# lenskit/lkpy

Hardware: AMD Instinct MI355X
Metric: ALS-implicit epochs/sec (ML-25M-shaped, k=64) (higher is better)
Workload: dtype f32; 1 GPU; MovieLens-25M-shaped, als-implicit k=64, 829 timed epochs, 1 x MI355X; solver=cholesky, n_items=62423, nnz=25000095, parallelism=single GPU

## Files before the change

### lkpy_amd/csrc/als_cg.hip

```cpp
#include "als_plan.h"
#include "common.h"

namespace lk {

template <int FPL>
struct Vec {
    float v[FPL];
};

template <int FPL>
__device__ __forceinline__ Vec<FPL> vload(const float *p)
{
    Vec<FPL> r;
    if constexpr (FPL == 1) {
        r.v[0] = p[0];
    } else if constexpr (FPL == 2) {
        f32x2 t = *reinterpret_cast<const f32x2 *>(p);
        r.v[0] = t.x;
        r.v[1] = t.y;
    } else {
        f32x4 t = *reinterpret_cast<const f32x4 *>(p);
        r.v[0] = t.x;
        r.v[1] = t.y;
        r.v[2] = t.z;
        r.v[3] = t.w;
    }
    return r;
}

template <int CTRL>
__device__ __forceinline__ float cg_dpp(float x)
{
    return __builtin_bit_cast(
        float, __builtin_amdgcn_update_dpp(0, __builtin_bit_cast(int, x), CTRL, 0xf, 0xf, false));
}
__device__ __forceinline__ float cg_wave_sum(float x)
{
    x += cg_dpp<0xB1>(x);
    x += cg_dpp<0x4E>(x);
    x += cg_dpp<0x141>(x);
    x += cg_dpp<0x140>(x);
    return (bcast(x, 0) + bcast(x, 16)) + (bcast(x, 32) + bcast(x, 48));
}
template <int FPL>
__device__ __forceinline__ float vdot(const Vec<FPL> &a, const Vec<FPL> &b)
{
    float s = 0.f;
#pragma unroll
    for (int c = 0; c < FPL; ++c) s = fmaf(a.v[c], b.v[c], s);
    return cg_wave_sum(s);
}

__device__ __forceinline__ int64_t cg_uniform64(int64_t v)
{
    const unsigned lo = __builtin_amdgcn_readfirstlane((unsigned)v);
    const unsigned hi = __builtin_amdgcn_readfirstlane((unsigned)((unsigned long long)v >> 32));
    return (int64_t)(((unsigned long long)hi << 32) | lo);
}

__device__ __forceinline__ float cg_reduce8(const float (&a)[8], int lane)
{
    const bool b0 = lane & 1, b1 = lane & 2, b2 = lane & 4;
    float b[4], c[2];
#pragma unroll
    for (int m = 0; m < 4; ++m) {
        const float keep = b0 ? a[m + 4] : a[m], send = b0 ? a[m] : a[m + 4];
        b[m] = keep + cg_dpp<0xB1>(send);
    }
#pragma unroll
    for (int m = 0; m < 2; ++m) {
        const float keep = b1 ? b[m + 2] : b[m], send = b1 ? b[m] : b[m + 2];
        c[m] = keep + cg_dpp<0x4E>(send);
    }
    const float keep = b2 ? c[1] : c[0], send = b2 ? c[0] : c[1];
    float d = keep + __shfl_xor(send, 4, 64);
    d += cg_dpp<0x128>(d);
    d += __shfl_xor(d, 16, 64);
    d += __shfl_xor(d, 32, 64);
    return d;
}
#define CG_REV3(j) ((((j) & 1) << 2) | ((j) & 2) | (((j) & 4) >> 2))

template <int KP, bool IS64, int NW>
__global__ __launch_bounds__(256, (NW == 1 && KP <= 128) ? 3 : 2) void als_cg_kernel(
    const typename IndPtr<IS64>::type *__restrict__ indptr, const int32_t *__restrict__ indices,
    const float *__restrict__ values, const int32_t *__restrict__ order, int64_t n_rows,
    const float *__restrict__ other, float *__restrict__ this_, const float *__restrict__ otor,
    int ld_otor, int k, float tol, int max_iter, float *__restrict__ row_delta,
    int *__restrict__ status, TaskCtlDev ctl, int64_t t_begin, int64_t t_end)
{
    static_assert(NW == 4 || NW == 1, "NW");
    constexpr int FPL = KP / 64;
    constexpr bool OTOR_LDS = KP <= 128;
    constexpr int GB = 8;
    constexpr int RI = 64 / FPL;
    constexpr int NG = RI / GB;
    constexpr int TB = FPL <= 2 ? 16 : 8;
    __shared__ float part[4][KP];
    extern __shared__ __attribute__((aligned(16))) float otor_s[];
    const int wave_in_wg = __builtin_amdgcn_readfirstlane(threadIdx.x >> 6);
    const int wave = NW == 4 ? wave_in_wg : 0;
    const bool lead = NW == 1 || wave_in_wg == 0;
    const int lane = lane_id();
    const int f0 = lane * FPL;
    auto team_sync = [&]() {
        if constexpr (NW == 4) __syncthreads();
    };
    const int myj = CG_REV3(lane & 7);
    if (OTOR_LDS) {
        for (int e = threadIdx.x; e < KP * KP; e += 256) {
            const int g = e / KP, f = e % KP;
            otor_s[e] = (g < k && f < k) ? otor[(int64_t)g * ld_otor + f] : 0.f;
        }
        __syncthreads();
    }

    __shared__ int s_cancel;
    (void)n_rows;
    for (int64_t t = t_begin + (NW == 4 ? (int64_t)blockIdx.x : (int64_t)blockIdx.x * 4 + wave_in_wg);
         t < t_end; t += (NW == 4 ? (int64_t)gridDim.x : (int64_t)gridDim.x * 4)) {
        if (NW == 4 && ctl.d_cancel) {
            if (threadIdx.x == 0) s_cancel = ctl_cancelled(ctl, (blockIdx.x & 31) == 0) ? 1 : 0;
            __syncthreads();
            const int c = s_cancel;
            __syncthreads();
            if (c) return;
        }
        const int row = __builtin_amdgcn_readfirstlane(order[t]);
        const int64_t beg = cg_uniform64(indptr[row]), end = cg_uniform64(indptr[row + 1]);
        float *xrow = this_ + (int64_t)row * KP;
        if (end == beg) {
            if (lead)
#pragma unroll
                for (int c = 0; c < FPL; ++c) xrow[f0 + c] = 0.f;
            if (lead && lane == 0) row_delta[row] = 0.f;
            if (ctl.d_done && lead && lane == 0) ctl_advance(ctl, 1);
            continue;
        }
        const int64_t n = end - beg;
        const int share = n >= NW * RI ? RI : (int)((n + NW * GB - 1) / (NW * GB)) * GB;
        const int64_t rbeg = beg + (int64_t)wave * share;
        int nres = (int)(end - rbeg < share ? end - rbeg : share);
        nres = __builtin_amdgcn_readfirstlane(nres < 0 ? 0 : nres);
        const int64_t sbeg = beg + NW * (int64_t)share;
        Vec<FPL> qres[RI];
        float vg[NG];
        const int myitem = indices[lane < nres ? rbeg + lane : beg];
#pragma unroll
        for (int g = 0; g < NG; ++g) {
            vg[g] = 0.f;
            if (g * GB < nres) {
                vg[g] = (g * GB + myj < nres) ? values[rbeg + g * GB + myj] : 0.f;
#pragma unroll
                for (int j = 0; j < GB; ++j) {
                    const int i = g * GB + j;
                    const int64_t it = __builtin_amdgcn_readlane(myitem, i);
                    qres[i] = vload<FPL>(other + it * KP + f0);
                    if (i >= nres)
#pragma unroll
                        for (int c = 0; c < FPL; ++c) qres[i].v[c] = 0.f;
                }
            } else {
#pragma unroll
                for (int j = 0; j < GB; ++j)
#pragma unroll
                    for (int c = 0; c < FPL; ++c) qres[g * GB + j].v[c] = 0.f;
            }
        }
        auto apply = [&](const Vec<FPL> &p, Vec<FPL> &out) {
            Vec<FPL> u;
#pragma unroll
            for (int c = 0; c < FPL; ++c) u.v[c] = 0.f;
#pragma unroll
            for (int g2 = 0; g2 < NG; g2 += 2) {
                if (g2 * GB < nres) {
                    float a[2][GB];
#pragma unroll
                    for (int h = 0; h < 2; ++h)
#pragma unroll
                        for (int j = 0; j < GB; ++j) {
                            float sacc = 0.f;
#pragma unroll
                            for (int c = 0; c < FPL; ++c)
                                sacc = fmaf(qres[(g2 + h) * GB + j].v[c], p.v[c], sacc);
                            a[h][j] = sacc;
                        }
                    float coefv[2];
#pragma unroll
                    for (int h = 0; h < 2; ++h) coefv[h] = vg[g2 + h] * cg_reduce8(a[h], lane);
#pragma unroll
                    for (int h = 0; h < 2; ++h)
#pragma unroll
                        for (int j = 0; j < GB; ++j) {
                            const float coef = bcast(coefv[h], CG_REV3(j));
#pragma unroll
                            for (int c = 0; c < FPL; ++c)
                                u.v[c] = fmaf(coef, qres[(g2 + h) * GB + j].v[c], u.v[c]);
                        }
                }
            }
            for (int64_t e0 = sbeg + (int64_t)wave * TB; e0 < end; e0 += NW * TB) {
                Vec<FPL> q[TB];
                const int tailitem = indices[(lane < TB && e0 + lane < end) ? e0 + lane : beg];
                float vmine[TB / GB];
#pragma unroll
                for (int h = 0; h < TB / GB; ++h)
                    vmine[h] = (e0 + h * GB + myj < end) ? values[e0 + h * GB + myj] : 0.f;
#pragma unroll
                for (int j = 0; j < TB; ++j) {
                    const int64_t it = __builtin_amdgcn_readlane(tailitem, j);
                    q[j] = vload<FPL>(other + it * KP + f0);
                }
#pragma unroll
                for (int h = 0; h < TB / GB; ++h) {
                    float a[GB];
#pragma unroll
                    for (int j = 0; j < GB; ++j) {
                        float sacc = 0.f;
#pragma unroll
                        for (int c = 0; c < FPL; ++c) sacc = fmaf(q[h * GB + j].v[c], p.v[c], sacc);
                        a[j] = sacc;
                    }
                    const float coefv = vmine[h] * cg_reduce8(a, lane);
#pragma unroll
                    for (int j = 0; j < GB; ++j) {
                        const float coef = bcast(coefv, CG_REV3(j));
#pragma unroll
                        for (int c = 0; c < FPL; ++c)
                            u.v[c] = fmaf(coef, q[h * GB + j].v[c], u.v[c]);
                    }
                }
            }
#pragma unroll 8
            for (int gi = 0; gi < KP / NW; ++gi) {
                const int g = wave * (KP / NW) + gi;
                if (!OTOR_LDS && g >= k) continue;
                float pg = 0.f;
#pragma unroll
                for (int c = 0; c < FPL; ++c)
                    if ((g % FPL) == c) pg = bcast(p.v[c], g / FPL);
                if (OTOR_LDS) {
                    const Vec<FPL> o = vload<FPL>(&otor_s[g * KP + f0]);
#pragma unroll
                    for (int c = 0; c < FPL; ++c) u.v[c] = fmaf(pg, o.v[c], u.v[c]);
                } else {
#pragma unroll
                    for (int c = 0; c < FPL; ++c) {
                        const int f = f0 + c;
                        const float o = (f < k) ? otor[(int64_t)g * ld_otor + f] : 0.f;
                        u.v[c] = fmaf(pg, o, u.v[c]);
                    }
                }
            }
            if constexpr (NW == 1) {
                out = u;
            } else {
                __syncthreads();
#pragma unroll
                for (int c = 0; c < FPL; ++c) part[wave][f0 + c] = u.v[c];
                __syncthreads();
#pragma unroll
                for (int c = 0; c < FPL; ++c)
                    out.v[c] = ((part[0][f0 + c] + part[1][f0 + c]) + part[2][f0 + c]) +
                               part[3][f0 + c];
            }
        };

        Vec<FPL> y, d;
        {
            Vec<FPL> yw, dw;
#pragma unroll
            for (int c = 0; c < FPL; ++c) yw.v[c] = dw.v[c] = 0.f;
#pragma unroll
            for (int g = 0; g < NG; ++g) {
                if (g * GB < nres) {
#pragma unroll
                    for (int j = 0; j < GB; ++j) {
                        const float val = bcast(vg[g], CG_REV3(j));
#pragma unroll
                        for (int c = 0; c < FPL; ++c) {
                            const float qc = qres[g * GB + j].v[c];
                            yw.v[c] = fmaf(val + 1.0f, qc, yw.v[c]);
                            dw.v[c] = fmaf(val * qc, qc, dw.v[c]);
                        }
                    }
                }
            }
            for (int64_t e0 = sbeg + (int64_t)wave * GB; e0 < end; e0 += NW * GB) {
                Vec<FPL> q[GB];
                float val[GB];
                const bool mine = lane < GB && e0 + lane < end;
                const int tailitem = indices[mine ? e0 + lane : beg];
                const float tailval = mine ? values[e0 + lane] : -1.0f;
#pragma unroll
                for (int j = 0; j < GB; ++j) {
                    const bool in = e0 + j < end;
                    const int64_t it = __builtin_amdgcn_readlane(tailitem, j);
                    val[j] = bcast(tailval, j);
                    q[j] = vload<FPL>(other + it * KP + f0);
                    if (!in)
#pragma unroll
                        for (int c = 0; c < FPL; ++c) q[j].v[c] = 0.f;
                }
#pragma unroll
                for (int j = 0; j < GB; ++j)
#pragma unroll
                    for (int c = 0; c < FPL; ++c) {
                        yw.v[c] = fmaf(val[j] + 1.0f, q[j].v[c], yw.v[c]);
                        dw.v[c] = fmaf(val[j] * q[j].v[c], q[j].v[c], dw.v[c]);
                    }
            }
            if constexpr (NW == 1) {
#pragma unroll
                for (int c = 0; c < FPL; ++c) {
                    const int f = f0 + c;
                    const float od = (f < k) ? otor[(int64_t)f * ld_otor + f] : 1.0f;
                    y.v[c] = yw.v[c];
                    d.v[c] = od + dw.v[c];
                }
            } else {
                __syncthreads();
#pragma unroll
                for (int c = 0; c < FPL; ++c) part[wave][f0 + c] = yw.v[c];
                __syncthreads();
#pragma unroll
                for (int c = 0; c < FPL; ++c)
                    y.v[c] = ((part[0][f0 + c] + part[1][f0 + c]) + part[2][f0 + c]) +
                             part[3][f0 + c];
                __syncthreads();
#pragma unroll
                for (int c = 0; c < FPL; ++c) part[wave][f0 + c] = dw.v[c];
                __syncthreads();
#pragma unroll
                for (int c = 0; c < FPL; ++c) {
                    const int f = f0 + c;
                    const float od = (f < k) ? otor[(int64_t)f * ld_otor + f] : 1.0f;
                    d.v[c] = od + (((part[0][f] + part[1][f]) + part[2][f]) + part[3][f]);
                }
            }
        }
        Vec<FPL> dinv;
#pragma unroll
        for (int c = 0; c < FPL; ++c) dinv.v[c] = 1.0f / d.v[c];
        Vec<FPL> x, xold, r, z, p, ap;
#pragma unroll
        for (int c = 0; c < FPL; ++c) xold.v[c] = x.v[c] = xrow[f0 + c];
        apply(x, ap);
        const float ynorm2 = vdot<FPL>(y, y);
#pragma unroll
        for (int c = 0; c < FPL; ++c) {
            r.v[c] = y.v[c] - ap.v[c];
            z.v[c] = r.v[c] * dinv.v[c];
            p.v[c] = z.v[c];
        }
        float rz = vdot<FPL>(r, z);
        float rr = vdot<FPL>(r, r);
        const float stop = tol * tol * ynorm2;
        int it = 0;
        bool bad = !(ynorm2 == ynorm2);
        while (it < max_iter && rr > stop && !bad) {
            apply(p, ap);
            const float pap = vdot<FPL>(p, ap);
            if (!(pap > 0.f)) {
                bad = true;
                break;
            }
            const float alpha = rz / pap;
#pragma unroll
            for (int c = 0; c < FPL; ++c) {
                x.v[c] = fmaf(alpha, p.v[c], x.v[c]);
                r.v[c] = fmaf(-alpha, ap.v[c], r.v[c]);
                z.v[c] = r.v[c] * dinv.v[c];
            }
            const float rz_new = vdot<FPL>(r, z);
            rr = vdot<FPL>(r, r);
            const float beta = rz_new / rz;
            rz = rz_new;
#pragma unroll
            for (int c = 0; c < FPL; ++c) p.v[c] = fmaf(beta, p.v[c], z.v[c]);
            ++it;
        }
        float dd = 0.f;
#pragma unroll
        for (int c = 0; c < FPL; ++c) {
            const float df = (f0 + c < k) ? x.v[c] - xold.v[c] : 0.f;
            dd = fmaf(df, df, dd);
            bad = bad || !(fabsf(x.v[c]) <= 3.0e38f);
        }
        dd = cg_wave_sum(dd);
        if (lead) {
#pragma unroll
            for (int c = 0; c < FPL; ++c) xrow[f0 + c] = (f0 + c < k) ? x.v[c] : 0.f;
            if (lane == 0) row_delta[row] = dd;
        }
        if (__any(bad) && lead && lane == 0) atomicCAS(status, 0, row + 1);
        if (lead && lane == 0) {
            atomicAdd(&status[2], it);
            atomicAdd(&status[3], 1);
        }
        if (ctl.d_done && lead && lane == 0) ctl_advance(ctl, 1);
        team_sync();
    }
}

template <int KP, bool IS64>
static int launch_cg(const lk_als_plan *p, const void *indptr, const int32_t *indices,
                     const float *values, int64_t n_rows, int k, float *this_,
                     const float *other, const float *otor, int ld_otor, char *ws,
                     float *out_frob, hipStream_t st, int64_t t_begin)
{
    using IT = typename IndPtr<IS64>::type;
    int *status = reinterpret_cast<int *>(ws + p->off_status);
    float *row_delta = reinterpret_cast<float *>(ws + p->off_delta);
    float *partial = reinterpret_cast<float *>(ws + p->off_partial);
    if (t_begin == 0) LK_HIP_CHECK(hipMemsetAsync(status, 0, 64, st));
    if (p->ctl) {
        LK_HIP_CHECK(hipMemsetAsync(row_delta, 0, (size_t)n_rows * sizeof(float), st));
        int rc = ctl_begin(p->ctl, n_rows, n_rows, st);
        if (rc != LK_OK) return rc;
    }
    const int max_iter = p->cg_max_iter > 0 ? p->cg_max_iter : k;
    int64_t t_w1 = p->ctl ? n_rows : p->t_cg1;
    if (t_w1 < t_begin) t_w1 = t_begin;
    const size_t lds = KP <= 128 ? (size_t)KP * KP * sizeof(float) : 0;
    auto k4 = als_cg_kernel<KP, IS64, 4>;
    auto k1 = als_cg_kernel<KP, IS64, 1>;
    if (lds > 0) {
        LK_HIP_CHECK(hipFuncSetAttribute(reinterpret_cast<const void *>(k4),
                                         hipFuncAttributeMaxDynamicSharedMemorySize, (int)lds));
        LK_HIP_CHECK(hipFuncSetAttribute(reinterpret_cast<const void *>(k1),
                                         hipFuncAttributeMaxDynamicSharedMemorySize, (int)lds));
    }
    if (t_w1 > t_begin) {
        const int64_t n4 = t_w1 - t_begin;
        const int64_t blocks = n4 < 256 * 8 ? n4 : 256 * 8;
        hipLaunchKernelGGL(k4, dim3((unsigned)blocks), dim3(256), lds, st,
                           static_cast<const IT *>(indptr), indices, values, p->d_order, n_rows,
                           other, this_, otor, ld_otor, k, p->cg_tol, max_iter, row_delta,
                           status, p->ctl ? p->ctl->dev() : TaskCtlDev{}, t_begin, t_w1);
    }
    if (n_rows > t_w1) {
        const int64_t n1 = (n_rows - t_w1 + 3) / 4;
        const int64_t blocks = n1 < 256 * 8 ? n1 : 256 * 8;
        hipLaunchKernelGGL(k1, dim3((unsigned)blocks), dim3(256), lds, st,
                           static_cast<const IT *>(indptr), indices, values, p->d_order, n_rows,
                           other, this_, otor, ld_otor, k, p->cg_tol, max_iter, row_delta,
                           status, TaskCtlDev{}, t_w1, n_rows);
    }
    return launch_delta_reduce(row_delta, n_rows, partial, out_frob, st);
}

int als_cg_half_epoch(const lk_als_plan *p, const void *indptr, int is64, const int32_t *indices,
                      const float *values, int64_t n_rows, int k, float *this_, int ld_this,
                      const float *other, int ld_other, const float *otor, int ld_otor, char *ws,
                      float *out_frob, hipStream_t st)
{
    int64_t t_begin = 0;
    const int64_t t_exact = p->ctl ? 0 : p->cg_exact;
    if (t_exact > 0) {
        p->dense_limit = t_exact;
        const int rc =
            p->KP > 64 ? als_blk_half_epoch(p, indptr, is64, indices, values, n_rows, 0, k, this_,
                                            other, otor, ld_otor, ws, out_frob, st, false, 0.f)
                       : als_chol_half_epoch(p, indptr, is64, indices, values, n_rows, k, this_,
                                             ld_this, other, ld_other, otor, ld_otor, ws, out_frob,
                                             st, false, 0.f);
        p->dense_limit = -1;
        if (rc != LK_OK) return rc;
        t_begin = t_exact;
    }
#define LK_CG_CASE(KPV)                                                                     \
    return is64 ? launch_cg<KPV, true>(p, indptr, indices, values, n_rows, k, this_, other, \
                                       otor, ld_otor, ws, out_frob, st, t_begin)            \
                : launch_cg<KPV, false>(p, indptr, indices, values, n_rows, k, this_, other, \
                                        otor, ld_otor, ws, out_frob, st, t_begin)
    switch (p->KP) {
        case 64: LK_CG_CASE(64);
        case 128: LK_CG_CASE(128);
        case 256: LK_CG_CASE(256);
    }
#undef LK_CG_CASE
    set_error("CG solver: unsupported padded embedding size %d (needs k > 32)", p->KP);
    return LK_E_INVALID;
}

}

extern "C" int lk_als_plan_cg_stats(const lk_als_plan *plan, void *d_ws, void *stream,
                                    int64_t *out_iterations, int64_t *out_rows)
{
    LK_REQUIRE(plan && d_ws, "lk_als_plan_cg_stats: null pointer");
    int st[4] = {0, 0, 0, 0};
    LK_HIP_CHECK(hipMemcpyAsync(st, static_cast<char *>(d_ws) + plan->off_status, sizeof(st),
                                hipMemcpyDeviceToHost, lk::as_stream(stream)));
    LK_HIP_CHECK(hipStreamSynchronize(lk::as_stream(stream)));
    if (out_iterations) *out_iterations = st[2];
    if (out_rows) *out_rows = st[3];
    return LK_OK;
}
```

### lkpy_amd/csrc/als_chol.hip

```cpp
#include <algorithm>
#include <utility>

#include "als_plan.h"
#include "common.h"
#include "delta_reduce.h"

#ifndef LK_ALS_RING
#define LK_ALS_RING 4
#endif

namespace lk {

#ifdef LK_ALS_PHASES
__device__ unsigned *lk_als_phase_buf;
#define LK_PHASE_T(var) const unsigned long long var = __builtin_amdgcn_s_memtime()
#define LK_PHASE_ADD(i, a, b) \
    if (lane_id() == 0 && lk_als_phase_buf) lk_als_phase_buf[t * 8 + (i)] = (unsigned)((b) - (a))
#else
#define LK_PHASE_T(var)
#define LK_PHASE_ADD(i, a, b)
#endif

__host__ __device__ constexpr int als_tiles(int NT) { return NT * (NT + 1) / 2; }
__host__ __device__ constexpr int tidx(int ti, int tj) { return tj * (tj + 1) / 2 + ti; }

template <int NT>
struct Gram {
    f32x4 t[als_tiles(NT)];
    float y[NT];
    float yc = 0.f;
};

__device__ __forceinline__ void swap32(float &a, float &b)
{
    asm volatile("s_nop 1\n\tv_permlane32_swap_b32 %0, %1" : "+v"(a), "+v"(b));
}
__device__ __forceinline__ void swap16(float &a, float &b)
{
    asm volatile("s_nop 1\n\tv_permlane16_swap_b32 %0, %1" : "+v"(a), "+v"(b));
}

template <int NT>
__device__ __forceinline__ void y_chain_step(float &yc, const float (&q)[NT], const float v1)
{
    float p[4];
#pragma unroll
    for (int t = 0; t < 4; ++t) p[t] = t < NT ? __fmul_rn(q[t < NT ? t : 0], v1) : 0.f;
    swap32(p[0], p[2]);
    swap32(p[1], p[3]);
    swap16(p[0], p[1]);
    swap16(p[2], p[3]);
    yc = __fadd_rn(yc, p[0]);
    yc = __fadd_rn(yc, p[1]);
    yc = __fadd_rn(yc, p[2]);
    yc = __fadd_rn(yc, p[3]);
}

template <int NT>
__device__ __forceinline__ void load_q(const float *p, float (&q)[NT])
{
    if constexpr (NT == 1) {
        q[0] = *p;
    } else if constexpr (NT == 2) {
        f32x2 t = *reinterpret_cast<const f32x2 *>(p);
        q[0] = t.x;
        q[1] = t.y;
    } else {
        static_assert(NT == 4, "Cholesky path supports NT in {1,2,4}");
        f32x4 t = *reinterpret_cast<const f32x4 *>(p);
        q[0] = t.x;
        q[1] = t.y;
        q[2] = t.z;
        q[3] = t.w;
    }
}

template <int NT>
struct GatherRing {
    static constexpr int RING = LK_ALS_RING;
    float q[RING][NT];
    float v[RING];
};

template <int NT>
__device__ __forceinline__ void ring_issue(GatherRing<NT> &R, const int slot_idx, const int g,
                                           const float *stage_slot,
                                           const float *__restrict__ other)
{
    constexpr int KP = NT * 16;
    const int lane = lane_id();
    const int col = __builtin_bit_cast(int, stage_slot[g * 4]);
    R.v[slot_idx] = stage_slot[64 + g * 4];
    load_q<NT>(other + (int64_t)col * KP + (lane & 15) * NT, R.q[slot_idx]);
}

template <int NT, bool MASKED, bool SEQY = false, bool WITH_Y = true>
__device__ __forceinline__ void ring_consume(Gram<NT> &G, const GatherRing<NT> &R,
                                             const int slot_idx, const int g, const int nb,
                                             const bool expl)
{
    const int lane = lane_id();
    const bool live = !MASKED || (g * 4 + (lane >> 4)) < nb;
    const float v = R.v[slot_idx];
    const float va = expl ? 1.0f : v;
    float q[NT], a[NT];
#pragma unroll
    for (int t = 0; t < NT; ++t) {
        q[t] = live ? R.q[slot_idx][t] : 0.f;
        a[t] = q[t] * va;
    }
#pragma unroll
    for (int tj = 0; tj < NT; ++tj)
#pragma unroll
        for (int ti = 0; ti <= tj; ++ti)
            G.t[tidx(ti, tj)] = __builtin_amdgcn_mfma_f32_16x16x4f32(a[ti], q[tj],
                                                                     G.t[tidx(ti, tj)], 0, 0, 0);
    if constexpr (WITH_Y) {
        const float v1 = expl ? v : v + 1.0f;
        if constexpr (SEQY) {
            y_chain_step<NT>(G.yc, q, v1);
        } else {
#pragma unroll
            for (int t = 0; t < NT; ++t) G.y[t] = fmaf(q[t], v1, G.y[t]);
        }
    }
}

constexpr int GRAM_STAGE_WORDS = 256;

template <int NT, bool SEQY = false, bool WITH_Y = true>
__device__ __forceinline__ void gram_accumulate(Gram<NT> &G, const int32_t *__restrict__ cols,
                                                const float *__restrict__ vals, int64_t beg,
                                                int64_t end, const float *__restrict__ other,
                                                int , const bool expl,
                                                float *stage )
{
    const int lane = lane_id();
    constexpr int RING = GatherRing<NT>::RING;
    static_assert(RING >= 1 && RING <= 8 && 16 % RING == 0, "gather ring: 1, 2, 4 or 8 slots");
    GatherRing<NT> R;
    const int64_t last = end - 1;

    float *wr_cur = stage + lane, *wr_nxt = stage + 128 + lane;
    const float *rd_cur = stage + (lane >> 4), *rd_nxt = stage + 128 + (lane >> 4);
    int nxt_col;
    float nxt_val;
    {
        const int64_t e = (beg + lane < end) ? beg + lane : last;
        wr_cur[0] = __builtin_bit_cast(float, cols[e]);
        wr_cur[64] = vals[e];
    }
#pragma unroll
    for (int g = 0; g < RING; ++g) ring_issue<NT>(R, g, g, rd_cur, other);

    int64_t base = beg;
    for (; base + 64 <= end; base += 64) {
        {
            const int64_t e = (base + 64 + lane < end) ? base + 64 + lane : last;
            nxt_col = cols[e];
            nxt_val = vals[e];
        }
#pragma unroll
        for (int g = 0; g < 16; ++g) {
            ring_consume<NT, false, SEQY, WITH_Y>(G, R, g % RING, g, 64, expl);
            if (g == 16 - RING - 2) {
                wr_nxt[0] = __builtin_bit_cast(float, nxt_col);
                wr_nxt[64] = nxt_val;
            }
            if (g < 16 - RING)
                ring_issue<NT>(R, g % RING, g + RING, rd_cur, other);
            else
                ring_issue<NT>(R, g % RING, g + RING - 16, rd_nxt, other);
            __builtin_amdgcn_sched_barrier(0);
        }
        float *tw = wr_cur;
        wr_cur = wr_nxt;
        wr_nxt = tw;
        const float *tr = rd_cur;
        rd_cur = rd_nxt;
        rd_nxt = tr;
    }
    if (base < end) {
        const int nb = (int)(end - base);
        const int ngroups = (nb + 3) >> 2;
#pragma unroll
        for (int g = 0; g < 16; ++g) {
            if (g < ngroups) ring_consume<NT, true, SEQY, WITH_Y>(G, R, g % RING, g, nb, expl);
            if (g < 16 - RING) ring_issue<NT>(R, g % RING, g + RING, rd_cur, other);
        }
    }
}

#ifndef LK_ALS_DMA_RING
#define LK_ALS_DMA_RING 8
#endif
constexpr int DMA_RING = LK_ALS_DMA_RING;

template <int N>
__device__ __forceinline__ void wait_vm()
{
    asm volatile("s_waitcnt vmcnt(%0)" ::"n"(N) : "memory");
}
__device__ __forceinline__ void wait_vm_upto(const int n)
{
    if (n >= 7) wait_vm<7>();
    else if (n == 6) wait_vm<6>();
    else if (n == 5) wait_vm<5>();
    else if (n == 4) wait_vm<4>();
    else if (n == 3) wait_vm<3>();
    else if (n == 2) wait_vm<2>();
    else if (n == 1) wait_vm<1>();
    else wait_vm<0>();
}

__device__ __forceinline__ void dma_issue(const unsigned ring_lds, const int slot_idx, const int g,
                                          const float *stage_slot,
                                          const float *__restrict__ other)
{
    const int lane = lane_id();
    const unsigned col = __builtin_bit_cast(unsigned, stage_slot[g * 4]);
    const uint64_t lane_base = (uint64_t)(uintptr_t)(other + (lane & 15) * 4);
    const float *src = reinterpret_cast<const float *>(lane_base + (uint64_t)col * 256ull);
    const unsigned dst = ring_lds + slot_idx * 1024;
    unsigned keep;
    asm volatile(
        "s_mov_b32 %0, m0\n\ts_mov_b32 m0, %2\n\ts_nop 0\n\t"
        "global_load_lds_dwordx4 %1, off\n\ts_mov_b32 m0, %0"
        : "=&s"(keep)
        : "v"(src), "s"(dst)
        : "memory");
}

struct DmaOperand {
    f32x4 q;
    float v;
};
__device__ __forceinline__ DmaOperand dma_fetch(const float *ring, const int slot_idx, const int g,
                                                const float *stage_slot)
{
    DmaOperand o;
    o.q = *reinterpret_cast<const f32x4 *>(ring + slot_idx * 256 + lane_id() * 4);
    o.v = stage_slot[64 + g * 4];
    return o;
}

template <bool MASKED, bool SEQY = false, bool WITH_Y = true>
__device__ __forceinline__ void dma_apply(Gram<4> &G, const DmaOperand &o, const int g,
                                          const int nb, const bool expl)
{
    const int lane = lane_id();
    const bool live = !MASKED || (g * 4 + (lane >> 4)) < nb;
    const float v = o.v;
    const float va = expl ? 1.0f : v;
    float q[4] = {o.q.x, o.q.y, o.q.z, o.q.w}, a[4];
#pragma unroll
    for (int t = 0; t < 4; ++t) {
        q[t] = live ? q[t] : 0.f;
        a[t] = q[t] * va;
    }
#pragma unroll
    for (int tj = 0; tj < 4; ++tj)
#pragma unroll
        for (int ti = 0; ti <= tj; ++ti)
            G.t[tidx(ti, tj)] = __builtin_amdgcn_mfma_f32_16x16x4f32(a[ti], q[tj],
                                                                     G.t[tidx(ti, tj)], 0, 0, 0);
    if constexpr (WITH_Y) {
        const float v1 = expl ? v : v + 1.0f;
        if constexpr (SEQY) {
            y_chain_step<4>(G.yc, q, v1);
        } else {
#pragma unroll
            for (int t = 0; t < 4; ++t) G.y[t] = fmaf(q[t], v1, G.y[t]);
        }
    }
}

template <bool MASKED, bool SEQY = false, bool WITH_Y = true>
__device__ __forceinline__ void dma_consume(Gram<4> &G, const float *ring, const int slot_idx,
                                            const int g, const int nb, const float *stage_slot,
                                            const bool expl)
{
    dma_apply<MASKED, SEQY, WITH_Y>(G, dma_fetch(ring, slot_idx, g, stage_slot), g, nb, expl);
}

template <int NT>
__host__ __device__ constexpr int slab_floats();
template <int NT, bool WITH_Y = true>
__device__ __forceinline__ void slab_store(const Gram<NT> &G, float *__restrict__ slab);
template <int NT, bool WITH_Y = true>
__device__ __forceinline__ void gram_zero(Gram<NT> &G);

template <bool SEQY = false, bool WITH_Y = true, int RING = DMA_RING>
__device__ __forceinline__ void gram_accumulate_dma(Gram<4> &G, const int32_t *__restrict__ cols,
                                                    const float *__restrict__ vals, int64_t beg,
                                                    int64_t end, const float *__restrict__ other,
                                                    const bool expl, float *ring, float *stage,
                                                    float *__restrict__ slab = nullptr)
{
    static_assert(RING == 8 || RING == 4, "DMA ring: 4 or 8 groups");
    const int lane = lane_id();
    const int64_t last = end - 1;
    const unsigned ring_lds =
        __builtin_amdgcn_readfirstlane((unsigned)(uintptr_t) reinterpret_cast<void *>(ring));

    float *wr_cur = stage + lane, *wr_nxt = stage + 128 + lane;
    const float *rd_cur = stage + (lane >> 4), *rd_nxt = stage + 128 + (lane >> 4);
    {
        const int64_t e = (beg + lane < end) ? beg + lane : last;
        wr_cur[0] = __builtin_bit_cast(float, cols[e]);
        wr_cur[64] = vals[e];
    }
    const int total = (int)((end - beg + 3) >> 2);
#pragma unroll
    for (int g = 0; g < RING; ++g)
        if (g < total) dma_issue(ring_lds, g, g, rd_cur, other);

    int64_t base = beg;
    int g0 = 0;
    for (; g0 + 16 + RING <= total; base += 64, g0 += 16) {
        int nxt_col;
        float nxt_val;
        {
            const int64_t e = (base + 64 + lane < end) ? base + 64 + lane : last;
            nxt_col = cols[e];
            nxt_val = vals[e];
        }
        wait_vm<RING - 1>();
        DmaOperand cur = dma_fetch(ring, 0, 0, rd_cur);
#pragma unroll
        for (int g = 0; g < 16; ++g) {
            DmaOperand nxt = cur;
            if (g + 1 < 16) {
                wait_vm<RING - 2>();
                nxt = dma_fetch(ring, (g + 1) % RING, g + 1, rd_cur);
            }
            dma_apply<false, SEQY, WITH_Y>(G, cur, g, 64, expl);
            if (g == 16 - RING - 2) {
                wr_nxt[0] = __builtin_bit_cast(float, nxt_col);
                wr_nxt[64] = nxt_val;
            }
            if (g < 16 - RING)
                dma_issue(ring_lds, g % RING, g + RING, rd_cur, other);
            else
                dma_issue(ring_lds, g % RING, g + RING - 16, rd_nxt, other);
            cur = nxt;
            __builtin_amdgcn_sched_barrier(0);
        }
        if (slab && ((g0 + 16) & 63) == 0) {
            slab_store<4, WITH_Y>(G, slab);
            slab += slab_floats<4>();
            gram_zero<4, WITH_Y>(G);
        }
        float *tw = wr_cur;
        wr_cur = wr_nxt;
        wr_nxt = tw;
        const float *tr = rd_cur;
        rd_cur = rd_nxt;
        rd_nxt = tr;
    }
    for (; g0 < total; base += 64, g0 += 16) {
        const int nb = (int)((end - base < 64) ? end - base : 64);
        const bool more = g0 + 16 < total;
        int nxt_col = 0;
        float nxt_val = 0.f;
        if (more) {
            const int64_t e = (base + 64 + lane < end) ? base + 64 + lane : last;
            nxt_col = cols[e];
            nxt_val = vals[e];
        }
#pragma unroll
        for (int g = 0; g < 16; ++g) {
            const int gg = g0 + g;
            if (gg < total) {
                const int later = total - 1 - gg;
                wait_vm_upto(later < RING - 1 ? later : RING - 1);
                dma_consume<true, SEQY, WITH_Y>(G, ring, g % RING, g, nb, rd_cur, expl);
            }
            if (g == 16 - RING - 2 && more) {
                wr_nxt[0] = __builtin_bit_cast(float, nxt_col);
                wr_nxt[64] = nxt_val;
            }
            if (gg + RING < total) {
                if (g < 16 - RING)
                    dma_issue(ring_lds, g % RING, g + RING, rd_cur, other);
                else
                    dma_issue(ring_lds, g % RING, g + RING - 16, rd_nxt, other);
            }
        }
        if (slab && ((g0 + 16) & 63) == 0 && g0 + 16 < total) {
            slab_store<4, WITH_Y>(G, slab);
            slab += slab_floats<4>();
            gram_zero<4, WITH_Y>(G);
        }
        float *tw = wr_cur;
        wr_cur = wr_nxt;
        wr_nxt = tw;
        const float *tr = rd_cur;
        rd_cur = rd_nxt;
        rd_nxt = tr;
    }
}

template <bool WITH_Y = true, int RING = DMA_RING>
__device__ __forceinline__ void gram_accumulate_dma_256(Gram<4> &G, const int32_t *__restrict__ cols,
                                                        const float *__restrict__ vals, int64_t beg,
                                                        const float *__restrict__ other,
                                                        const bool expl, float *ring, float *stage)
{
    constexpr int TOTAL = 64;
    const int lane = lane_id();
    const unsigned ring_lds =
        __builtin_amdgcn_readfirstlane((unsigned)(uintptr_t) reinterpret_cast<void *>(ring));
    float *const wr0 = stage + lane, *const wr1 = stage + 128 + lane;
    const float *const rd0 = stage + (lane >> 4), *const rd1 = stage + 128 + (lane >> 4);
    wr0[0] = __builtin_bit_cast(float, cols[beg + lane]);
    wr0[64] = vals[beg + lane];
#pragma unroll
    for (int g = 0; g < RING; ++g) dma_issue(ring_lds, g, g, rd0, other);
#pragma unroll
    for (int b = 0; b < 4; ++b) {
        float *const wr_nxt = (b & 1) ? wr0 : wr1;
        const float *const rd_cur = (b & 1) ? rd1 : rd0, *const rd_nxt = (b & 1) ? rd0 : rd1;
        int nxt_col = 0;
        float nxt_val = 0.f;
        if (b < 3) {
            nxt_col = cols[beg + 64 * (b + 1) + lane];
            nxt_val = vals[beg + 64 * (b + 1) + lane];
        }
        {
            const int later = TOTAL - 1 - 16 * b;
            wait_vm_upto(later < RING - 1 ? later : RING - 1);
        }
        DmaOperand cur = dma_fetch(ring, 0, 0, rd_cur);
#pragma unroll
        for (int g = 0; g < 16; ++g) {
            const int gg = 16 * b + g;
            DmaOperand nxt = cur;
            if (g + 1 < 16) {
                const int later = TOTAL - 1 - (gg + 1);
                const int issued_after = (gg + RING < TOTAL ? gg + RING - 1 : TOTAL - 1) - (gg + 1);
                wait_vm_upto(issued_after < later ? issued_after : later);
                nxt = dma_fetch(ring, (g + 1) % RING, g + 1, rd_cur);
            }
            dma_apply<false, false, WITH_Y>(G, cur, g, 64, expl);
            if (g == 16 - RING - 2 && b < 3) {
                wr_nxt[0] = __builtin_bit_cast(float, nxt_col);
                wr_nxt[64] = nxt_val;
            }
            if (gg + RING < TOTAL) {
                if (g < 16 - RING)
                    dma_issue(ring_lds, g % RING, g + RING, rd_cur, other);
                else
                    dma_issue(ring_lds, g % RING, g + RING - 16, rd_nxt, other);
            }
            cur = nxt;
            __builtin_amdgcn_sched_barrier(0);
        }
    }
}

template <int NT>
__host__ __device__ constexpr int slab_floats()
{
    return (als_tiles(NT) * 4 + NT) * 64;
}

template <int NT, bool WITH_Y>
__device__ __forceinline__ void slab_store(const Gram<NT> &G, float *__restrict__ slab)
{
    const int lane = lane_id();
#pragma unroll
    for (int e = 0; e < als_tiles(NT); ++e)
        __builtin_nontemporal_store(G.t[e], reinterpret_cast<f32x4 *>(slab + (e * 64 + lane) * 4));
    if constexpr (WITH_Y) {
#pragma unroll
        for (int t = 0; t < NT; ++t) slab[als_tiles(NT) * 256 + lane * NT + t] = G.y[t];
    }
}

template <int NT, bool WITH_Y = true>
__device__ __forceinline__ void slab_add(Gram<NT> &G, const float *__restrict__ slab)
{
    const int lane = lane_id();
#pragma unroll
    for (int e = 0; e < als_tiles(NT); ++e)
        G.t[e] += *reinterpret_cast<const f32x4 *>(slab + (e * 64 + lane) * 4);
    if constexpr (WITH_Y) {
#pragma unroll
        for (int t = 0; t < NT; ++t) G.y[t] += slab[als_tiles(NT) * 256 + lane * NT + t];
    }
}

template <int NT, bool WITH_Y>
__device__ __forceinline__ void gram_zero(Gram<NT> &G)
{
#pragma unroll
    for (int e = 0; e < als_tiles(NT); ++e) G.t[e] = f32x4{0.f, 0.f, 0.f, 0.f};
    if constexpr (WITH_Y) {
#pragma unroll
        for (int t = 0; t < NT; ++t) G.y[t] = 0.f;
    }
}

__global__ __launch_bounds__(256) void slab_group_reduce_kernel(float *__restrict__ slabs,
                                                                int64_t slab_floats,
                                                                int64_t sum_floats,
                                                                const int32_t *__restrict__ grp_head,
                                                                const int32_t *__restrict__ grp_cnt,
                                                                int parts)
{
    const int g = blockIdx.x / parts;
    const int64_t e = ((int64_t)(blockIdx.x - g * parts) * 256 + threadIdx.x) * 4;
    if (e >= sum_floats) return;
    float *head = slabs + (size_t)grp_head[g] * slab_floats + e;
    const int cnt = grp_cnt[g];
    f32x4 acc = *reinterpret_cast<const f32x4 *>(head);
    int c = 1;
    for (; c + 8 <= cnt; c += 8) {
        f32x4 v[8];
#pragma unroll
        for (int u = 0; u < 8; ++u)
            v[u] = __builtin_nontemporal_load(
                reinterpret_cast<const f32x4 *>(head + (size_t)(c + u) * slab_floats));
#pragma unroll
        for (int u = 0; u < 8; ++u) acc += v[u];
    }
    for (; c < cnt; ++c)
        acc += *reinterpret_cast<const f32x4 *>(head + (size_t)c * slab_floats);
    *reinterpret_cast<f32x4 *>(head) = acc;
}

int launch_slab_group_reduce(const lk_als_plan *p, float *slabs, size_t slab_floats, hipStream_t st,
                             size_t sum_floats)
{
    if (p->n_groups <= 0) return LK_OK;
    if (sum_floats == 0) sum_floats = slab_floats;
    const int parts = (int)((sum_floats / 4 + 255) / 256);
    hipLaunchKernelGGL(slab_group_reduce_kernel, dim3((unsigned)(p->n_groups * parts)), dim3(256),
                       0, st, slabs, (int64_t)slab_floats, (int64_t)sum_floats, p->d_grp_head,
                       p->d_grp_cnt, parts);
    LK_HIP_CHECK(hipGetLastError());
    return LK_OK;
}

#ifndef LK_ALS_CHUNK_RING
#define LK_ALS_CHUNK_RING 8
#endif
constexpr int CHUNK_RING = LK_ALS_CHUNK_RING;

template <int NT>
__host__ __device__ constexpr int chunk_lds_floats()
{
    return GRAM_STAGE_WORDS + (NT == 4 ? CHUNK_RING * 256 : 0);
}

int als_chol_chunk_wgs_per_cu()
{
    const int by_lds = (int)(160 * 1024 / (4 * chunk_lds_floats<4>() * sizeof(float)));
    return by_lds < 5 ? by_lds : 5;
}

template <int NT, bool EXPL, bool WITH_Y>
__device__ __forceinline__ void als_chunk_body(
    const int32_t *__restrict__ indices, const float *__restrict__ values,
    const int64_t *__restrict__ chunk_beg, const int32_t *__restrict__ chunk_len,
    int64_t n_chunks, const float *__restrict__ other, int ld, float *__restrict__ slabs,
    const int64_t blk, float *__restrict__ lds_flat,
    const int32_t *__restrict__ chunk_slab = nullptr, const int block_len = 0)
{
    constexpr bool DMA = NT == 4;
    float(*stage_all)[chunk_lds_floats<NT>()] =
        reinterpret_cast<float(*)[chunk_lds_floats<NT>()]>(lds_flat);
    const int wave = __builtin_amdgcn_readfirstlane(threadIdx.x >> 6);
    const int64_t c = blk * 4 + wave;
    if (c >= n_chunks) return;
    Gram<NT> G;
    gram_zero<NT, WITH_Y>(G);
    const int64_t beg = chunk_beg[c];
    float *slab = slabs + (size_t)(chunk_slab ? chunk_slab[c] : c) * slab_floats<NT>();
    if constexpr (DMA) {
        const int len = chunk_len[c];
        if (block_len == 256 && len > 256) {
            gram_accumulate_dma<false, WITH_Y, CHUNK_RING>(
                G, indices, values, beg, beg + len, other, EXPL,
                stage_all[wave] + GRAM_STAGE_WORDS, stage_all[wave], slab);
            slab += (size_t)((len - 1) >> 8) * slab_floats<NT>();
        } else if (len == 256)
            gram_accumulate_dma_256<WITH_Y, CHUNK_RING>(
                G, indices, values, beg, other, EXPL, stage_all[wave] + GRAM_STAGE_WORDS,
                stage_all[wave]);
        else
            gram_accumulate_dma<false, WITH_Y, CHUNK_RING>(
                G, indices, values, beg, beg + len, other, EXPL,
                stage_all[wave] + GRAM_STAGE_WORDS, stage_all[wave]);
    } else
        gram_accumulate<NT, false, WITH_Y>(G, indices, values, beg, beg + chunk_len[c], other, ld,
                                           EXPL, stage_all[wave]);
    slab_store<NT, WITH_Y>(G, slab);
}

template <int NT, bool EXPL, bool WITH_Y>
__global__ __launch_bounds__(256) void als_chunk_kernel(
    const int32_t *__restrict__ indices, const float *__restrict__ values,
    const int64_t *__restrict__ chunk_beg, const int32_t *__restrict__ chunk_len,
    int64_t n_chunks, const float *__restrict__ other, int ld, float *__restrict__ slabs,
    const int32_t *__restrict__ chunk_slab, int block_len)
{
    __shared__ __attribute__((aligned(16))) float lds_flat[4 * chunk_lds_floats<NT>()];
    als_chunk_body<NT, EXPL, WITH_Y>(indices, values, chunk_beg, chunk_len, n_chunks, other, ld,
                                     slabs, (int64_t)blockIdx.x, lds_flat, chunk_slab, block_len);
}

template <int KP>
struct LPack {
    __host__ __device__ static constexpr int c0(int j) { return (j + 1) & ~3; }
    __host__ __device__ static constexpr int off(int j)
    {
        const int m = j >> 2, r = j & 3;
        return 4 * KP * m - 8 * m * m + 4 * m + r * (KP - 4 * m);
    }
    static constexpr int SIZE = KP * KP / 2 + KP;
};

template <int NT>
__host__ __device__ constexpr int hybrid_lds_floats()
{
    return LPack<NT * 16>::SIZE + NT * 16 + 256;
}

template <int NT, int M>
__device__ __forceinline__ void hybrid_step(Gram<NT> &G, float &b, float &minpiv,
                                            float *__restrict__ lds, const int lane)
{
    constexpr int KP = NT * 16, J = 4 * M, TJ = M >> 2, MG = M & 3;
    using P = LPack<KP>;
    const int slot = lane >> 4;
    float *rinvarr = lds + P::SIZE;
    float *scr = rinvarr + KP;

#pragma unroll
    for (int t = TJ; t < NT; ++t)
        if (slot == MG)
            *reinterpret_cast<f32x4 *>(&scr[(t * 16 + (lane & 15)) * 4]) = G.t[tidx(TJ, t)];
    f32x4 pv = f32x4{0.f, 0.f, 0.f, 0.f};
    if (slot >= TJ && lane < KP) pv = *reinterpret_cast<const f32x4 *>(&scr[lane * 4]);
    float pr[4] = {pv.x, pv.y, pv.z, pv.w};

    float lp[4];
#pragma unroll
    for (int s0 = 0; s0 < 4; ++s0) {
        const int j = J + s0;
        const float piv = bcast(pr[s0], j);
        minpiv = fminf(minpiv, piv);
        const float rinv = __builtin_amdgcn_rsqf(piv);
        rinvarr[j] = rinv;
        const float lj = (lane > j) ? pr[s0] * rinv : 0.f;
        if (j + 1 < KP) {
            const bool in = lane >= P::c0(j) && lane < KP;
            float *dst = in ? &lds[P::off(j) + lane - P::c0(j)] : &scr[lane];
            *dst = lj;
        }
        const float zj = bcast(b, j) * rinv;
        b = fmaf(-lj, zj, b);
#pragma unroll
        for (int s = s0 + 1; s < 4; ++s) pr[s] = fmaf(-lj, bcast(lj, J + s), pr[s]);
        lp[s0] = lj;
    }
    if constexpr (J + 4 < KP) {
        swap32(lp[0], lp[2]);
        swap32(lp[1], lp[3]);
        swap16(lp[0], lp[1]);
        swap16(lp[2], lp[3]);
        float nq[NT];
#pragma unroll
        for (int t = TJ; t < NT; ++t) nq[t] = -lp[t];
#pragma unroll
        for (int ti = TJ; ti < NT; ++ti)
#pragma unroll
            for (int t2 = ti; t2 < NT; ++t2)
                G.t[tidx(ti, t2)] = __builtin_amdgcn_mfma_f32_16x16x4f32(
                    nq[ti], lp[t2], G.t[tidx(ti, t2)], 0, 0, 0);
    }
}

template <int NT, int... Ms>
__device__ __forceinline__ void hybrid_steps(Gram<NT> &G, float &b, float &minpiv,
                                             float *__restrict__ lds, const int lane,
                                             std::integer_sequence<int, Ms...>)
{
    (hybrid_step<NT, Ms>(G, b, minpiv, lds, lane), ...);
}

template <int NT>
__device__ __forceinline__ float hybrid_solve(Gram<NT> &G, float &b, float *__restrict__ lds
#ifdef LK_ALS_PHASES
                                              ,
                                              unsigned long long *tmid
#endif
)
{
    constexpr int KP = NT * 16;
    using P = LPack<KP>;
    int lane = lane_id();
    asm volatile("" : "+v"(lane));
    b = 0.f;
#pragma unroll
    for (int tt = 0; tt < NT; ++tt) b = ((lane >> 4) == tt) ? G.y[tt] : b;
    float minpiv = 3.0e38f;
    hybrid_steps<NT>(G, b, minpiv, lds, lane, std::make_integer_sequence<int, KP / 4>{});
#ifdef LK_ALS_PHASES
    asm volatile("" : "+v"(b));
    *tmid = __builtin_amdgcn_s_memtime();
#endif
    const float dinv = (lane < KP) ? lds[P::SIZE + lane] : 0.f;
    b *= dinv;
    const int my_c0 = (lane + 1) & ~3;
    const float *mycol = lds + P::off(lane) - my_c0;
#pragma unroll
    for (int j4 = KP / 4 - 1; j4 >= 0; --j4) {
        f32x4 l4 = f32x4{0.f, 0.f, 0.f, 0.f};
        if (lane < KP - 1 && 4 * j4 >= my_c0) l4 = *reinterpret_cast<const f32x4 *>(mycol + 4 * j4);
#pragma unroll
        for (int u = 3; u >= 0; --u) {
            const int j = 4 * j4 + u;
            if (j >= 1) {
                const float xj = bcast(b * dinv, j);
                b = fmaf(-l4[u], xj, b);
            }
        }
    }
    b *= dinv;
    return minpiv;
}

template <int NT, bool IS64, bool EXPL, bool CTL, bool YREF = false, bool SEQY = false>
__device__ __forceinline__ void als_solve_body(
    const typename IndPtr<IS64>::type *__restrict__ indptr, const int32_t *__restrict__ indices,
    const float *__restrict__ values, const int32_t *__restrict__ order, int64_t n_rows,
    const int32_t *__restrict__ row_slab, const float *__restrict__ other, int ld_other,
    float *__restrict__ this_, int ld_this, const float *__restrict__ otor_p,
    const float *__restrict__ slabs, float *__restrict__ row_delta, int *__restrict__ status,
    int k, float reg, TaskCtlDev ctl, const float *__restrict__ y_ref, int chunk_rt,
    const int64_t blk, float *__restrict__ lds_flat)
{
    constexpr int KP = NT * 16;
    float(*lds_all)[hybrid_lds_floats<NT>()] =
        reinterpret_cast<float(*)[hybrid_lds_floats<NT>()]>(lds_flat);

    const int wave = __builtin_amdgcn_readfirstlane(threadIdx.x >> 6);
    const int lane = lane_id();
    const int sub = lane & 15, slot = lane >> 4;
    const int64_t t = blk * 4 + wave;
    if (t >= n_rows) return;
    LK_PHASE_T(ph0);
    if constexpr (CTL) {
        int c = 0;
        if (lane == 0) c = ctl_cancelled(ctl, (blk & 63) == 0 && wave == 0) ? 1 : 0;
        if (__builtin_amdgcn_readfirstlane(c)) return;
    }
    const int row = order[t];
    const int64_t beg = indptr[row], end = indptr[row + 1];
    float *lds = lds_all[wave];

    const int my_f = (lane & 15) * NT + (lane >> 4);
    const bool my_valid = (lane < KP) && (my_f < k);
    float *xrow = this_ + (int64_t)row * ld_this;

    if (end == beg) {
        if (lane < KP) xrow[lane] = 0.f;
        if (lane == 0) row_delta[row] = 0.f;
        if constexpr (CTL)
            if (lane == 0) ctl_advance(ctl, 1);
        return;
    }

    LK_PHASE_T(ph1);
    Gram<NT> G;
#pragma unroll
    for (int tj = 0; tj < NT; ++tj)
#pragma unroll
        for (int ti = 0; ti <= tj; ++ti)
#pragma unroll
            for (int r = 0; r < 4; ++r)
                G.t[tidx(ti, tj)][r] = otor_p[(ti * 16 + slot * 4 + r) * KP + tj * 16 + sub];
#pragma unroll
    for (int tt = 0; tt < NT; ++tt) G.y[tt] = 0.f;

    const int first_slab = row_slab[row];
    if (first_slab >= 0) {
        const int64_t n = end - beg;
        const bool refo = YREF && chunk_rt > 0;
        const int ch = refo ? chunk_rt : LK_ALS_CHUNK;
        const int ns = (int)((n + ch - 1) / ch);
        const int step = refo ? ns : (ns > LK_ALS_SLAB_GROUP ? LK_ALS_SLAB_GROUP : 1);
        for (int s = 0; s < ns; s += step)
            slab_add<NT, !YREF>(G, slabs + (size_t)(first_slab + s) * slab_floats<NT>());
    } else {
        if constexpr (NT == 4)
            gram_accumulate_dma<SEQY && !YREF>(G, indices, values, beg, end, other, EXPL, lds,
                                               lds + LPack<KP>::SIZE + KP);
        else
            gram_accumulate<NT, SEQY && !YREF>(G, indices, values, beg, end, other, ld_other,
                                               EXPL, lds);
    }
    if (EXPL) {
        const float dg = reg * (float)(end - beg);
#pragma unroll
        for (int ti = 0; ti < NT; ++ti)
#pragma unroll
            for (int r = 0; r < 4; ++r)
                if (slot * 4 + r == sub && (slot * 4 + r) * NT + ti < k) G.t[tidx(ti, ti)][r] += dg;
    }

#ifdef LK_ALS_PHASES
    asm volatile("" : "+v"(G.t[0]), "+v"(G.t[als_tiles(NT) - 1]));
#endif
    LK_PHASE_T(ph2);
    if (SEQY && !YREF && first_slab < 0) {
#pragma unroll
        for (int tt = 0; tt < NT; ++tt) G.y[tt] = __shfl(G.yc, sub + 16 * tt, 64);
    } else {
#pragma unroll
        for (int tt = 0; tt < NT; ++tt) {
            G.y[tt] += __shfl_xor(G.y[tt], 16, 64);
            G.y[tt] += __shfl_xor(G.y[tt], 32, 64);
        }
    }
    if constexpr (YREF) {
#pragma unroll
        for (int tt = 0; tt < NT; ++tt) G.y[tt] = y_ref[(int64_t)t * KP + sub * NT + tt];
    }
    const float old = my_valid ? xrow[my_f] : 0.f;
    float b;
#ifdef LK_ALS_PHASES
    LK_PHASE_T(ph3);
    unsigned long long ph4 = 0;
    const float minpiv = hybrid_solve<NT>(G, b, lds, &ph4);
    asm volatile("" : "+v"(b));
    LK_PHASE_T(ph5);
#else
    const float minpiv = hybrid_solve<NT>(G, b, lds);
#endif
    const bool bad = !(minpiv > 0.f) || (my_valid && !(fabsf(b) <= 3.0e38f));
    if (__any(bad) && lane == 0) atomicCAS(status, 0, row + 1);

    float d = 0.f;
    if (my_valid) {
        xrow[my_f] = b;
        d = b - old;
    }
    const float d2 = wave_sum(d * d);
    if (lane == 0) row_delta[row] = d2;
    if constexpr (CTL)
        if (lane == 0) ctl_advance(ctl, 1);
#ifdef LK_ALS_PHASES
    LK_PHASE_T(ph6);
    LK_PHASE_ADD(0, ph0, ph1);
    LK_PHASE_ADD(1, ph1, ph2);
    LK_PHASE_ADD(2, ph2, ph3);
    LK_PHASE_ADD(3, ph3, ph4);
    LK_PHASE_ADD(4, ph4, ph5);
    LK_PHASE_ADD(5, ph5, ph6);
    LK_PHASE_ADD(6, (unsigned long long)beg, (unsigned long long)end);
    LK_PHASE_ADD(7, ph0, ph6);
#endif
}

template <int NT, bool IS64, bool EXPL, bool CTL, bool YREF = false, bool SEQY = false>
__global__ __launch_bounds__(256) __attribute__((amdgpu_waves_per_eu(4))) void als_solve_kernel(
    const typename IndPtr<IS64>::type *__restrict__ indptr, const int32_t *__restrict__ indices,
    const float *__restrict__ values, const int32_t *__restrict__ order, int64_t n_rows,
    const int32_t *__restrict__ row_slab, const float *__restrict__ other, int ld_other,
    float *__restrict__ this_, int ld_this, const float *__restrict__ otor_p,
    const float *__restrict__ slabs, float *__restrict__ row_delta, int *__restrict__ status,
    int k, float reg, TaskCtlDev ctl, const float *__restrict__ y_ref = nullptr,
    int chunk_rt = 0)
{
    __shared__ __attribute__((aligned(16))) float lds_flat[4 * hybrid_lds_floats<NT>()];
    als_solve_body<NT, IS64, EXPL, CTL, YREF, SEQY>(indptr, indices, values, order, n_rows,
                                                    row_slab, other, ld_other, this_, ld_this,
                                                    otor_p, slabs, row_delta, status, k, reg, ctl,
                                                    y_ref, chunk_rt, (int64_t)blockIdx.x, lds_flat);
}

template <int CTRL>
__device__ __forceinline__ float wb_dpp_add(float x)
{
    const int y = __builtin_amdgcn_update_dpp(0, __builtin_bit_cast(int, x), CTRL, 0xf, 0xf, false);
    return x + __builtin_bit_cast(float, y);
}
__device__ __forceinline__ float wb_row16_sum(float x)
{
    x = wb_dpp_add<0xB1>(x);
    x = wb_dpp_add<0x4E>(x);
    x = wb_dpp_add<0x141>(x);
    x = wb_dpp_add<0x140>(x);
    return x;
}

template <int KP, bool IS64>
__global__ __launch_bounds__(256) void als_wb64_kernel(
    const typename IndPtr<IS64>::type *__restrict__ indptr, const int32_t *__restrict__ indices,
    const float *__restrict__ values, const int32_t *__restrict__ order, int64_t n_tasks,
    const float *__restrict__ other, const float *__restrict__ z, float *__restrict__ this_,
    float *__restrict__ row_delta, int *__restrict__ status)
{
    constexpr int QF = KP / 4;
    constexpr int NQ = QF / 4;
    __shared__ __attribute__((aligned(16))) float lds_all[4][hybrid_lds_floats<4>()];
    const int wave = __builtin_amdgcn_readfirstlane(threadIdx.x >> 6);
    const int lane = lane_id();
    const int s = lane >> 4, c = lane & 15;
    const int64_t task = (int64_t)blockIdx.x * 4 + wave;
    if (task >= n_tasks) return;
    if (status[1] != 0) return;
    const int row = order[task];
    const int64_t beg = indptr[row], end = indptr[row + 1];
    const int n = (int)(end - beg);
    float *xrow = this_ + (int64_t)row * KP;
    float *lds = lds_all[wave];
    const int nte = __builtin_amdgcn_readfirstlane((n + 15) >> 4);

    const float *mrow[4], *zrow[4];
    float w[4], sv[4];
#pragma unroll
    for (int t = 0; t < 4; ++t) {
        const int el = 16 * t + c;
        const int64_t e = beg + (el < n ? el : n - 1);
        const int col = indices[e];
        const float v = el < n ? values[e] : 0.f;
        w[t] = el < n ? v + 1.0f : 0.f;
        sv[t] = __builtin_sqrtf(v);
        mrow[t] = other + (int64_t)col * KP + 4 * s;
        zrow[t] = z + (int64_t)col * KP + 4 * s;
    }
    f32x4 acc[4][4];
#pragma unroll
    for (int ti = 0; ti < 4; ++ti)
#pragma unroll
        for (int tj = 0; tj < 4; ++tj) acc[ti][tj] = f32x4{0.f, 0.f, 0.f, 0.f};
    for (int q = 0; q < NQ; ++q) {
        f32x4 mq[4], zq[4];
#pragma unroll
        for (int t = 0; t < 4; ++t) {
            mq[t] = f32x4{0.f, 0.f, 0.f, 0.f};
            zq[t] = f32x4{0.f, 0.f, 0.f, 0.f};
            if (t < nte) {
                mq[t] = *reinterpret_cast<const f32x4 *>(mrow[t] + 16 * q);
                zq[t] = *reinterpret_cast<const f32x4 *>(zrow[t] + 16 * q);
            }
        }
#pragma unroll
        for (int ti = 0; ti < 4; ++ti)
#pragma unroll
            for (int tj = 0; tj < 4; ++tj)
                if (ti < nte && tj < nte) {
#pragma unroll
                    for (int el = 0; el < 4; ++el)
                        acc[ti][tj] = __builtin_amdgcn_mfma_f32_16x16x4f32(
                            mq[ti][el], zq[tj][el], acc[ti][tj], 0, 0, 0);
                }
    }
    float b;
    float minpiv;
    auto build = [&](auto &G, auto ntc) {
        constexpr int NTS = decltype(ntc)::value;
#pragma unroll
        for (int ti = 0; ti < NTS; ++ti) {
            float svr[4], rhs[4];
#pragma unroll
            for (int r = 0; r < 4; ++r) {
                svr[r] = __shfl(sv[ti], 4 * s + r, 64);
                float r0 = 0.f;
#pragma unroll
                for (int tj = 0; tj < NTS; ++tj) r0 += wb_row16_sum(acc[ti][tj][r] * w[tj]);
                rhs[r] = svr[r] * r0;
            }
#pragma unroll
            for (int tj = ti; tj < NTS; ++tj)
#pragma unroll
                for (int r = 0; r < 4; ++r)
                    G.t[tidx(ti, tj)][r] = svr[r] * sv[tj] * acc[ti][tj][r] +
                                           ((ti == tj && (4 * s + r) == c) ? 1.0f : 0.f);
            float sel = rhs[0];
            sel = (c & 3) == 1 ? rhs[1] : sel;
            sel = (c & 3) == 2 ? rhs[2] : sel;
            sel = (c & 3) == 3 ? rhs[3] : sel;
            G.y[ti] = __shfl(sel, (c >> 2) * 16 + c, 64);
        }
    };
#ifdef LK_ALS_PHASES
    unsigned long long tmid_unused = 0;
#endif
    if (nte <= 2) {
        Gram<2> G;
        build(G, std::integral_constant<int, 2>{});
#ifdef LK_ALS_PHASES
        minpiv = hybrid_solve<2>(G, b, lds, &tmid_unused);
#else
        minpiv = hybrid_solve<2>(G, b, lds);
#endif
    } else {
        Gram<4> G;
        build(G, std::integral_constant<int, 4>{});
#ifdef LK_ALS_PHASES
        minpiv = hybrid_solve<4>(G, b, lds, &tmid_unused);
#else
        minpiv = hybrid_solve<4>(G, b, lds);
#endif
    }
    float g[4];
    bool bad = !(minpiv > 0.f);
#pragma unroll
    for (int t = 0; t < 4; ++t) {
        g[t] = t < nte ? w[t] - sv[t] * __shfl(b, 16 * t + c, 64) : 0.f;
        bad = bad || !(fabsf(g[t]) <= 3.0e38f);
    }
    if (__any(bad) && lane == 0) atomicCAS(status, 0, row + 1);
    float d2 = 0.f;
    for (int q = 0; q < NQ; ++q) {
        f32x4 a4 = f32x4{0.f, 0.f, 0.f, 0.f};
#pragma unroll
        for (int t = 0; t < 4; ++t)
            if (t < nte) {
                const f32x4 zq = *reinterpret_cast<const f32x4 *>(zrow[t] + 16 * q);
                a4.x = fmaf(g[t], zq.x, a4.x);
                a4.y = fmaf(g[t], zq.y, a4.y);
                a4.z = fmaf(g[t], zq.z, a4.z);
                a4.w = fmaf(g[t], zq.w, a4.w);
            }
        f32x4 xs;
        xs.x = wb_row16_sum(a4.x);
        xs.y = wb_row16_sum(a4.y);
        xs.z = wb_row16_sum(a4.z);
        xs.w = wb_row16_sum(a4.w);
        if (c == 0) {
            f32x4 *dst = reinterpret_cast<f32x4 *>(xrow + 4 * s + 16 * q);
            const f32x4 old = *dst;
            *dst = xs;
            const f32x4 d = xs - old;
            d2 += d.x * d.x + d.y * d.y + d.z * d.z + d.w * d.w;
        }
    }
    d2 = wave_sum(d2);
    if (lane == 0) row_delta[row] = d2;
}

int als_wb64_launch(const lk_als_plan *p, const void *indptr, int is64, const int32_t *indices,
                    const float *values, int64_t t0, int64_t t1, float *this_,
                    const float *other, const float *z, float *row_delta, int *status,
                    hipStream_t st)
{
    const int64_t n = t1 - t0;
    if (n <= 0) return LK_OK;
    const dim3 grid((unsigned)((n + 3) / 4)), block(256);
#define LK_WB64(KPV, IS)                                                                        \
    hipLaunchKernelGGL((als_wb64_kernel<KPV, IS>), grid, block, 0, st,                          \
                       static_cast<const typename IndPtr<IS>::type *>(indptr), indices, values, \
                       p->d_order + t0, n, other, z, this_, row_delta, status)
    if (p->KP == 256) {
        if (is64)
            LK_WB64(256, true);
        else
            LK_WB64(256, false);
    } else if (p->KP == 128) {
        if (is64)
            LK_WB64(128, true);
        else
            LK_WB64(128, false);
    } else {
        set_error("Woodbury row solve: unsupported padded embedding size %d", p->KP);
        return LK_E_INVALID;
    }
#undef LK_WB64
    LK_HIP_CHECK(hipGetLastError());
    return LK_OK;
}

template <int NT>
__global__ void als_prep_otor_kernel(const float *__restrict__ otor, int ld_otor, int k,
                                     float *__restrict__ otor_p)
{
    constexpr int KP = NT * 16;
    int idx = blockIdx.x * blockDim.x + threadIdx.x;
    if (idx >= KP * KP) return;
    int pr = idx / KP, pc = idx % KP;
    int fr = (pr & 15) * NT + (pr >> 4), fc = (pc & 15) * NT + (pc >> 4);
    float v;
    if (fr < k && fc < k)
        v = otor ? otor[fr * ld_otor + fc] : 0.f;
    else
        v = (pr == pc) ? 1.0f : 0.0f;
    otor_p[idx] = v;
}

__global__ void delta_partial_kernel(const float *__restrict__ row_delta, int64_t n,
                                     float *__restrict__ partial)
{
    __shared__ float sm[256];
    delta_partial_body(row_delta, n, (int)gridDim.x, (int)blockIdx.x, sm, partial);
}

__global__ void delta_final_kernel(const float *__restrict__ partial, int n,
                                   float *__restrict__ out)
{
    __shared__ float sm[256];
    delta_final_body(partial, n, sm, out);
}

constexpr int DELTA_BLOCKS = LK_DELTA_BLOCKS;

int launch_delta_reduce(const float *row_delta, int64_t n_rows, float *partial, float *out_frob,
                        hipStream_t st)
{
    hipLaunchKernelGGL(delta_partial_kernel, dim3(DELTA_BLOCKS), dim3(256), 0, st, row_delta,
                       n_rows, partial);
    hipLaunchKernelGGL(delta_final_kernel, dim3(1), dim3(256), 0, st, partial, DELTA_BLOCKS,
                       out_frob);
    LK_HIP_CHECK(hipGetLastError());
    return LK_OK;
}

template <int NT, bool IS64, bool EXPL>
struct CholKind {};

struct CholHalf {
    const lk_als_plan *p;
    const void *indptr;
    bool is64;
    const int32_t *indices;
    const float *values;
    int64_t n_rows;
    int k;
    float *this_;
    int ld_this;
    const float *other;
    int ld_other;
    char *ws;
    float reg;
    hipStream_t st;
    hipStream_t sr = nullptr;
    int64_t n_solve = 0, n_y = 0;
    float *yref = nullptr;
    bool tm = false;
    bool forked = false;

    int *status() const { return reinterpret_cast<int *>(ws + p->off_status); }
    float *otor_p() const { return reinterpret_cast<float *>(ws + p->off_otor); }
    float *row_delta() const { return reinterpret_cast<float *>(ws + p->off_delta); }
    float *partial() const { return reinterpret_cast<float *>(ws + p->off_partial); }
    float *slabs() const { return reinterpret_cast<float *>(ws + p->off_slabs); }
    ~CholHalf()
    {
        if (forked) (void)plan_join_rhs(p, st);
    }
};

template <int NT, bool IS64, bool EXPL>
static int chol_prep(CholHalf &h, CholKind<NT, IS64, EXPL>, const float *otor, int ld_otor)
{
    constexpr int KP = NT * 16;
    const lk_als_plan *p = h.p;
    LK_REQUIRE(!p->ref_order || (p->d_yref && !p->ctl),
               "a reference-order ALS plan needs its rhs workspace (lk_als_plan_set_rhs_workspace) "
               "and no task-control block");
    LK_HIP_CHECK(hipMemsetAsync(h.status(), 0, 64, h.st));
    if (p->ctl) {
        LK_HIP_CHECK(hipMemsetAsync(h.row_delta(), 0, (size_t)h.n_rows * sizeof(float), h.st));
        int rc = ctl_begin(p->ctl, h.n_rows, h.n_rows, h.st);
        if (rc != LK_OK) return rc;
    }
    hipLaunchKernelGGL(als_prep_otor_kernel<NT>, dim3((KP * KP + 255) / 256), dim3(256), 0, h.st,
                       otor, ld_otor, h.k, h.otor_p());
    LK_HIP_CHECK(hipGetLastError());
    return LK_OK;
}

template <int NT, bool IS64, bool EXPL>
static int chol_front(CholHalf &h, CholKind<NT, IS64, EXPL>)
{
    const lk_als_plan *p = h.p;
    hipStream_t st = h.st;
    float *slabs = h.slabs();
    h.tm = p->timing && p->timing_n < lk_als_plan::TIMING_RING;
    if (h.tm) LK_HIP_CHECK(hipEventRecord(p->ev[p->timing_n][0], st));
    h.n_solve = p->dense_limit >= 0 && p->dense_limit < h.n_rows ? p->dense_limit : h.n_rows;
    h.yref = p->hybrid ? reinterpret_cast<float *>(h.ws + p->off_yref)
                       : (p->ctl ? nullptr : p->d_yref);
    h.n_y = !h.yref ? 0 : (p->hybrid ? std::min<int64_t>(p->n_long, h.n_solve) : h.n_solve);
    h.sr = st;
    if (h.n_y > 0) {
        int rc = plan_fork_rhs(p, st, &h.sr);
        if (rc != LK_OK) return rc;
        h.forked = h.sr != st;
    }
    const bool chunk_y = !(h.yref != nullptr && h.n_y >= p->n_long);
    if (p->n_chunks > 0) {
#define LK_CHUNK_LAUNCH(WITHY)                                                                  \
    hipLaunchKernelGGL((als_chunk_kernel<NT, EXPL, WITHY>),                                    \
                       dim3((unsigned)((p->n_chunks + 3) / 4)), dim3(256), 0, st, h.indices,   \
                       h.values, p->d_chunk_beg, p->d_chunk_len, p->n_chunks, h.other,         \
                       h.ld_other, slabs, p->d_chunk_slab, p->unit > p->chunk ? (int)p->chunk : 0)
        if (chunk_y)
            LK_CHUNK_LAUNCH(true);
        else
            LK_CHUNK_LAUNCH(false);
#undef LK_CHUNK_LAUNCH
    }
    if (h.n_y > 0) {
        int rc = launch_rhs_reference(p, h.indptr, IS64 ? 1 : 0, h.indices, h.values, p->d_order,
                                      h.n_y, h.other, EXPL, h.yref, h.sr);
        if (rc != LK_OK) return rc;
    }
    if (p->n_chunks > 0) {
        hipStream_t sg = st;
        if (h.forked) {
            int rc = plan_rhs_wait_main(p, st);
            if (rc != LK_OK) return rc;
            sg = h.sr;
        }
        int rc = launch_slab_group_reduce(p, slabs, slab_floats<NT>(), sg,
                                          chunk_y ? 0 : (size_t)als_tiles(NT) * 256);
        if (rc != LK_OK) return rc;
    }
    if (h.tm) LK_HIP_CHECK(hipEventRecord(p->ev[p->timing_n][1], st));
    LK_HIP_CHECK(hipGetLastError());
    return LK_OK;
}

template <int NT, bool IS64, bool EXPL>
static int chol_solve(CholHalf &h, CholKind<NT, IS64, EXPL>, hipEvent_t otor_ready)
{
    const lk_als_plan *p = h.p;
    hipStream_t st = h.st;
    using IT = typename IndPtr<IS64>::type;
    const IT *ip = static_cast<const IT *>(h.indptr);
    const int ref_chunk = (p->ref_order || p->hybrid) ? p->chunk : 0;
    const int64_t n_y = h.n_y, n_solve = h.n_solve;
    float *yref = h.yref;
    if (otor_ready) LK_HIP_CHECK(hipStreamWaitEvent(st, otor_ready, 0));
#define LK_SOLVE_LAUNCH(CTLV, YREFV, T0, NTASKS, YPTR, STREAM)                                \
    LK_SOLVE_LAUNCH_S(CTLV, YREFV, false, T0, NTASKS, YPTR, STREAM)
#define LK_SOLVE_LAUNCH_S(CTLV, YREFV, SEQV, T0, NTASKS, YPTR, STREAM)                        \
    hipLaunchKernelGGL((als_solve_kernel<NT, IS64, EXPL, CTLV, YREFV, SEQV>),                  \
                       dim3((unsigned)(((NTASKS) + 3) / 4)), dim3(256), 0, (STREAM), ip,       \
                       h.indices, h.values, p->d_order + (T0), (NTASKS), p->d_row_slab,        \
                       h.other, h.ld_other, h.this_, h.ld_this, h.otor_p(), h.slabs(),         \
                       h.row_delta(), h.status(), h.k, h.reg,                                  \
                       (CTLV) ? p->ctl->dev() : TaskCtlDev{}, (YPTR), ref_chunk)
    const bool seqy = p->hybrid || p->ref_order;
    if (n_solve > n_y) {
        if (p->ctl) {
            if (seqy)
                LK_SOLVE_LAUNCH_S(true, false, true, n_y, n_solve - n_y, nullptr, st);
            else
                LK_SOLVE_LAUNCH(true, false, n_y, n_solve - n_y, nullptr, st);
        } else {
            if (seqy)
                LK_SOLVE_LAUNCH_S(false, false, true, n_y, n_solve - n_y, nullptr, st);
            else
                LK_SOLVE_LAUNCH(false, false, n_y, n_solve - n_y, nullptr, st);
        }
    }
    if (n_y > 0) {
        if (p->ctl) {
            h.forked = false;
            int rc = plan_join_rhs(p, st);
            if (rc != LK_OK) return rc;
            LK_SOLVE_LAUNCH(true, true, 0, n_y, yref, st);
        } else {
            if (otor_ready && h.sr != st) LK_HIP_CHECK(hipStreamWaitEvent(h.sr, otor_ready, 0));
            LK_SOLVE_LAUNCH(false, true, 0, n_y, yref, h.sr);
            h.forked = false;
            int rc = plan_join_rhs(p, st);
            if (rc != LK_OK) return rc;
        }
    }
#undef LK_SOLVE_LAUNCH
#undef LK_SOLVE_LAUNCH_S
    if (h.tm) {
        LK_HIP_CHECK(hipEventRecord(p->ev[p->timing_n][2], st));
        p->timing_n++;
    }
    LK_HIP_CHECK(hipGetLastError());
    return LK_OK;
}

template <class F>
static int chol_dispatch(const CholHalf &h, bool expl, F &&f)
{
    auto by_model = [&](auto nt, auto wide) {
        constexpr int NT = decltype(nt)::value;
        constexpr bool IS64 = decltype(wide)::value;
        return expl ? f(CholKind<NT, IS64, true>{}) : f(CholKind<NT, IS64, false>{});
    };
    auto by_width = [&](auto nt) {
        return h.is64 ? by_model(nt, std::true_type{}) : by_model(nt, std::false_type{});
    };
    switch (h.p->NT) {
        case 1: return by_width(std::integral_constant<int, 1>{});
        case 2: return by_width(std::integral_constant<int, 2>{});
        case 4: return by_width(std::integral_constant<int, 4>{});
    }
    set_error("%s: no Cholesky kernel for padded k=%d",
              expl ? "lk_als_explicit_half_epoch" : "lk_als_implicit_half_epoch", h.p->KP);
    return LK_E_INVALID;
}

static int half_prep(CholHalf &h, bool expl, const float *otor, int ld_otor)
{
    return chol_dispatch(h, expl, [&](auto kind) { return chol_prep(h, kind, otor, ld_otor); });
}

static int half_front(CholHalf &h, bool expl)
{
    return chol_dispatch(h, expl, [&](auto kind) { return chol_front(h, kind); });
}

static int half_solve(CholHalf &h, bool expl, hipEvent_t otor_ready)
{
    return chol_dispatch(h, expl, [&](auto kind) { return chol_solve(h, kind, otor_ready); });
}

size_t als_chol_slab_floats(int NT) { return (size_t)(als_tiles(NT) * 4 + NT) * 64; }

int als_chol_half_epoch(const lk_als_plan *p, const void *indptr, int is64, const int32_t *indices,
                        const float *values, int64_t n_rows, int k, float *this_, int ld_this,
                        const float *other, int ld_other, const float *otor, int ld_otor, char *ws,
                        float *out_frob, hipStream_t st, bool expl, float reg)
{
    CholHalf h{p, indptr, is64 != 0, indices, values, n_rows, k, this_, ld_this, other, ld_other, ws, reg, st};
    int rc = half_prep(h, expl, otor, ld_otor);
    if (rc == LK_OK) rc = half_front(h, expl);
    if (rc == LK_OK) rc = half_solve(h, expl, nullptr);
    if (rc != LK_OK) return rc;
    return launch_delta_reduce(h.row_delta(), n_rows, h.partial(), out_frob, st);
}

int als_chol_epoch(const lk_als_plan *pu, const lk_als_plan *pi, const void *u_indptr,
                   const int32_t *u_indices, const float *u_values, const void *i_indptr,
                   const int32_t *i_indices, const float *i_values, float *P, float *Q,
                   float *qtq, int ld_qtq, float user_reg, float *ptp, int ld_ptp, float item_reg,
                   char *ws_u, char *ws_i, float *gram_ws, float *out_delta, hipStream_t st)
{
    const int k = pu->k, KP = pu->KP;
    CholHalf hu{pu, u_indptr, pu->is64 != 0, u_indices, u_values, pu->n_rows, k, P, KP, Q, KP, ws_u, 0.f, st};
    CholHalf hi{pi, i_indptr, pi->is64 != 0, i_indices, i_values, pi->n_rows, k, Q, KP, P, KP, ws_i, 0.f, st};
    int rc = half_prep(hu, false, qtq, ld_qtq);
    if (rc == LK_OK) rc = half_front(hu, false);
    if (rc == LK_OK) rc = half_solve(hu, false, nullptr);
    if (rc != LK_OK) return rc;
    hipStream_t tu = st;
    rc = plan_fork_rhs(pu, st, &tu);
    if (rc != LK_OK) return rc;
    hu.forked = tu != st;
    rc = gramian_tail(P, pu->n_rows, k, KP, item_reg, ptp, ld_ptp, gram_ws, hu.row_delta(),
                      hu.partial(), out_delta, hi.otor_p(), hi.status(), tu);
    if (rc != LK_OK) return rc;
    hipEvent_t tail_u = nullptr;
    if (tu != st) {
        LK_HIP_CHECK(hipEventRecord(pu->ev_tail_rhs, tu));
        tail_u = pu->ev_tail_rhs;
    }
    rc = half_front(hi, false);
    if (rc == LK_OK) rc = half_solve(hi, false, tail_u);
    if (rc != LK_OK) return rc;
    hu.forked = false;
    return gramian_tail(Q, pi->n_rows, k, KP, user_reg, qtq, ld_qtq, gram_ws, hi.row_delta(),
                        hi.partial(), out_delta + 1, nullptr, nullptr, st);
}

}


#ifdef LK_ALS_PHASES
extern "C" int lk_als_phase_set(void *d_buf)
{
    LK_HIP_CHECK(hipDeviceSynchronize());
    LK_HIP_CHECK(hipMemcpyToSymbol(HIP_SYMBOL(lk::lk_als_phase_buf), &d_buf, sizeof(void *)));
    return LK_OK;
}
#endif
```

### lkpy_amd/csrc/als_plan.h

```cpp
#pragma once
#include <hip/hip_runtime.h>
#include <stdint.h>

#define LK_DELTA_BLOCKS 256

#ifndef LK_ALS_WB64_K128_DEFAULT
#define LK_ALS_WB64_K128_DEFAULT 64
#endif

#ifndef LK_ALS_CHUNK
#define LK_ALS_CHUNK 1024
#endif
#ifndef LK_ALS_LONG_ROW
#define LK_ALS_LONG_ROW 2048
#endif
#define LK_ALS_CHUNK_BLK LK_ALS_CHUNK
#ifndef LK_ALS_SLAB_GROUP
#define LK_ALS_SLAB_GROUP 16
#endif

struct lk_als_plan {
    int64_t n_rows = 0;
    int32_t k = 0, KP = 0, NT = 0, solver = 0;
    int32_t is64 = 0;
    int64_t n_chunks = 0;
    int64_t n_long = 0;
    int64_t t_short = 0;
    int64_t t_wb128 = 0, t_wb64 = 0, t_wb8 = 0, t_wb4 = 0;
    int64_t wb_rows = 0;
    int64_t cg_exact = 0;
    int64_t t_cg1 = 0;
    bool side_streams = true;
    bool chunk_dma = false;
    int device = -1;
    mutable const float *d_z = nullptr;
    float *d_zbuf = nullptr;
    const int *d_zflag_src = nullptr;
    bool z_for_others = false;
    float *d_yref = nullptr;
    bool ref_order = false;
    bool hybrid = false;
    size_t off_yref = 0;
    int32_t chunk = LK_ALS_CHUNK;
    int32_t unit = LK_ALS_CHUNK;
    int64_t n_slabs = 0;
    int32_t *d_chunk_slab = nullptr;
    int32_t long_row = LK_ALS_LONG_ROW;
    size_t off_ginv = 0, off_invws = 0;
    char *d_pack = nullptr;
    size_t pack_cap = 0;
    int32_t *d_order = nullptr;
    int32_t *d_row_slab = nullptr;
    int32_t *d_chunk_row = nullptr;
    int64_t *d_chunk_beg = nullptr;
    int32_t *d_chunk_len = nullptr;
    int64_t n_groups = 0;
    int32_t *d_grp_head = nullptr;
    int32_t *d_grp_cnt = nullptr;
    size_t off_status = 0, off_otor = 0, off_delta = 0, off_partial = 0, off_slabs = 0,
           ws_bytes = 0;
    mutable int64_t dense_limit = -1;
    struct lk_task_ctl *ctl = nullptr;
    float cg_tol = 1e-7f;
    int32_t cg_max_iter = 0;
    static constexpr int TIMING_RING = 128;
    bool timing = false;
    mutable int timing_n = 0;
    mutable hipEvent_t ev[TIMING_RING][3] = {};
    mutable hipStream_t side = nullptr;
    mutable hipEvent_t ev_fork = nullptr, ev_join = nullptr;
    mutable hipStream_t side_rhs = nullptr;
    mutable hipEvent_t ev_fork_rhs = nullptr, ev_join_rhs = nullptr, ev_mid_rhs = nullptr;
    mutable hipEvent_t ev_tail_rhs = nullptr;
};

namespace lk {
size_t als_chol_slab_floats(int NT);
int als_chol_half_epoch(const lk_als_plan *p, const void *indptr, int is64, const int32_t *indices,
                        const float *values, int64_t n_rows, int k, float *this_, int ld_this,
                        const float *other, int ld_other, const float *otor, int ld_otor, char *ws,
                        float *out_frob, hipStream_t st, bool expl, float reg);
size_t als_blk_slab_floats(int NT);
int als_blk_half_epoch(const lk_als_plan *p, const void *indptr, int is64, const int32_t *indices,
                       const float *values, int64_t n_rows, int64_t n_cols, int k, float *this_,
                       const float *other, const float *otor, int ld_otor, char *ws,
                       float *out_frob, hipStream_t st, bool expl, float reg);
size_t als_big_scratch_bytes(int KP, int64_t n_rows);
int als_big_half_epoch(const lk_als_plan *p, const void *indptr, int is64, const int32_t *indices,
                       const float *values, int64_t n_rows, int k, float *this_,
                       const float *other, const float *otor, int ld_otor, char *ws,
                       float *out_frob, hipStream_t st, bool expl, float reg);
int als_cg_half_epoch(const lk_als_plan *p, const void *indptr, int is64, const int32_t *indices,
                      const float *values, int64_t n_rows, int k, float *this_, int ld_this,
                      const float *other, int ld_other, const float *otor, int ld_otor, char *ws,
                      float *out_frob, hipStream_t st);
size_t gramian_big_workspace_bytes(int KP);
int gramian_big(const float *m, int64_t n, int k, int KP, float reg, float *out, int ld_out,
                float *ws, hipStream_t st);
int als_wb_launch(const lk_als_plan *p, const void *indptr, int is64, const int32_t *indices,
                  const float *values, int64_t t0, int64_t n_rows, float *this_,
                  const float *other, const float *z, float *row_delta, int *status,
                  hipStream_t st);
int als_wb4_launch(const lk_als_plan *p, const void *indptr, int is64, const int32_t *indices,
                   const float *values, int64_t t0, int64_t n_rows, float *this_,
                   const float *other, const float *z, float *row_delta, int *status,
                   hipStream_t st, int slots = 4);
int als_wb64_launch(const lk_als_plan *p, const void *indptr, int is64, const int32_t *indices,
                    const float *values, int64_t t0, int64_t t1, float *this_,
                    const float *other, const float *z, float *row_delta, int *status,
                    hipStream_t st);
size_t spd_inverse_workspace_bytes(int KP);
int spd_inverse(const float *a, int lda, int k, int KP, float *out, int *flag, void *ws,
                hipStream_t st);
int launch_rhs_reference(const lk_als_plan *p, const void *indptr, int is64,
                         const int32_t *indices, const float *values, const int32_t *order,
                         int64_t n_tasks, const float *other, bool expl, float *y_out,
                         hipStream_t st);
int plan_fork_rhs(const lk_als_plan *p, hipStream_t st, hipStream_t *side);
int plan_join_rhs(const lk_als_plan *p, hipStream_t st);
int plan_rhs_wait_main(const lk_als_plan *p, hipStream_t st);
int launch_slab_group_reduce(const lk_als_plan *p, float *slabs, size_t slab_floats, hipStream_t st,
                             size_t sum_floats = 0);
int als_chol_chunk_wgs_per_cu();
int launch_delta_reduce(const float *row_delta, int64_t n_rows, float *partial, float *out_frob,
                        hipStream_t st);
int gramian_tail(const float *m, int64_t n, int k, int KP, float reg, float *out, int ld_out,
                 float *gram_ws, const float *row_delta, float *partial, float *out_delta,
                 float *next_otor_p, int *next_status, hipStream_t st);
int als_chol_epoch(const lk_als_plan *pu, const lk_als_plan *pi, const void *u_indptr,
                   const int32_t *u_indices, const float *u_values, const void *i_indptr,
                   const int32_t *i_indices, const float *i_values, float *P, float *Q,
                   float *qtq, int ld_qtq, float user_reg, float *ptp, int ld_ptp, float item_reg,
                   char *ws_u, char *ws_i, float *gram_ws, float *out_delta, hipStream_t st);
}
```

### lkpy_amd/csrc/als_plan.hip

```cpp
#include <stdlib.h>
#include <string.h>
#include <strings.h>

#include <algorithm>
#include <initializer_list>
#include <mutex>
#include <vector>

#include "als_plan.h"
#include "common.h"

namespace lk {

int plan_fork_rhs(const lk_als_plan *p, hipStream_t st, hipStream_t *side)
{
    *side = st;
    if (!p->side_streams) return LK_OK;
    if (!p->side_rhs) {
        p->side_rhs = lk::side_stream_acquire();
        LK_REQUIRE(p->side_rhs != nullptr, "als: no side stream");
        LK_HIP_CHECK(hipEventCreateWithFlags(&p->ev_fork_rhs, hipEventDisableTiming));
        LK_HIP_CHECK(hipEventCreateWithFlags(&p->ev_join_rhs, hipEventDisableTiming));
        LK_HIP_CHECK(hipEventCreateWithFlags(&p->ev_mid_rhs, hipEventDisableTiming));
        LK_HIP_CHECK(hipEventCreateWithFlags(&p->ev_tail_rhs, hipEventDisableTiming));
    }
    LK_HIP_CHECK(hipEventRecord(p->ev_fork_rhs, st));
    LK_HIP_CHECK(hipStreamWaitEvent(p->side_rhs, p->ev_fork_rhs, 0));
    *side = p->side_rhs;
    return LK_OK;
}

int plan_rhs_wait_main(const lk_als_plan *p, hipStream_t st)
{
    if (!p->side_rhs) return LK_OK;
    LK_HIP_CHECK(hipEventRecord(p->ev_mid_rhs, st));
    LK_HIP_CHECK(hipStreamWaitEvent(p->side_rhs, p->ev_mid_rhs, 0));
    return LK_OK;
}

int plan_join_rhs(const lk_als_plan *p, hipStream_t st)
{
    if (!p->side_rhs) return LK_OK;
    LK_HIP_CHECK(hipEventRecord(p->ev_join_rhs, p->side_rhs));
    LK_HIP_CHECK(hipStreamWaitEvent(st, p->ev_join_rhs, 0));
    return LK_OK;
}

}

extern "C" int32_t lk_padded_dim(int32_t k)
{
    if (k < 1) return 0;
    if (k <= 16) return 16;
    if (k <= 32) return 32;
    if (k <= 64) return 64;
    if (k <= 128) return 128;
    if (k <= 256) return 256;
    if (k <= 1024) return (k + 63) / 64 * 64;
    return 0;
}

namespace {
struct PackPool {
    static constexpr int SLOTS = 8;
    static constexpr size_t MAX_BYTES = (size_t)8 << 20;
    std::mutex mu;
    struct Slot {
        char *ptr = nullptr;
        size_t cap = 0;
        int dev = -1;
    } slot[SLOTS];
};
PackPool &pack_pool()
{
    static PackPool pool;
    return pool;
}
char *pack_pool_take(size_t bytes, size_t *cap)
{
    if (bytes > PackPool::MAX_BYTES) return nullptr;
    int dev = -1;
    if (hipGetDevice(&dev) != hipSuccess) return nullptr;
    PackPool &pl = pack_pool();
    std::lock_guard<std::mutex> lock(pl.mu);
    int best = -1;
    for (int i = 0; i < PackPool::SLOTS; ++i)
        if (pl.slot[i].ptr && pl.slot[i].dev == dev && pl.slot[i].cap >= bytes &&
            (best < 0 || pl.slot[i].cap < pl.slot[best].cap))
            best = i;
    if (best < 0) return nullptr;
    char *ptr = pl.slot[best].ptr;
    *cap = pl.slot[best].cap;
    pl.slot[best].ptr = nullptr;
    return ptr;
}
bool pack_pool_give(char *ptr, size_t cap)
{
    if (cap > PackPool::MAX_BYTES) return false;
    int dev = -1;
    if (hipGetDevice(&dev) != hipSuccess) return false;
    PackPool &pl = pack_pool();
    std::lock_guard<std::mutex> lock(pl.mu);
    for (int i = 0; i < PackPool::SLOTS; ++i)
        if (!pl.slot[i].ptr) {
            pl.slot[i].ptr = ptr;
            pl.slot[i].cap = cap;
            pl.slot[i].dev = dev;
            return true;
        }
    return false;
}
}

static bool switch_on(const char *name)
{
    const char *e = getenv(name);
    return !(e && e[0] == '0');
}

static int device_cu_count(int dev)
{
    static std::mutex mu;
    static int known[64] = {};
    std::lock_guard<std::mutex> lock(mu);
    const bool slot = dev >= 0 && dev < 64;
    if (slot && known[dev] > 0) return known[dev];
    int n = 0;
    if (dev < 0 ||
        hipDeviceGetAttribute(&n, hipDeviceAttributeMultiprocessorCount, dev) != hipSuccess || n < 0)
        n = 0;
    if (slot) known[dev] = n;
    return n;
}

extern "C" int lk_als_plan_create_ex(lk_als_plan **out, const void *h_indptr, int indptr_is_64,
                                     int64_t n_rows, int32_t k, int32_t solver, int32_t flags);

extern "C" int lk_als_plan_create(lk_als_plan **out, const void *h_indptr, int indptr_is_64,
                                  int64_t n_rows, int32_t k, int32_t solver)
{
    const char *e = getenv("LK_ALS_RHS_ORDER");
    int32_t flags = LK_ALS_PLAN_HYBRID_ORDER;
    if (e && e[0]) {
        if (!strcasecmp(e, "accurate")) flags = 0;
        else if (!strcasecmp(e, "reference")) flags = LK_ALS_PLAN_REFERENCE_ORDER;
        else
            LK_REQUIRE(!strcasecmp(e, "auto") || !strcasecmp(e, "hybrid") || !strcasecmp(e, "default"),
                       "lk_als_plan_create: unknown LK_ALS_RHS_ORDER '%s' (auto / reference / accurate)",
                       e);
    }
    return lk_als_plan_create_ex(out, h_indptr, indptr_is_64, n_rows, k, solver, flags);
}

extern "C" int lk_als_plan_create_ex(lk_als_plan **out, const void *h_indptr, int indptr_is_64,
                                     int64_t n_rows, int32_t k, int32_t solver, int32_t flags)
{
    LK_REQUIRE(out != nullptr && h_indptr != nullptr, "lk_als_plan_create: null pointer");
    LK_REQUIRE((flags & ~(LK_ALS_PLAN_REFERENCE_ORDER | LK_ALS_PLAN_HYBRID_ORDER)) == 0,
               "lk_als_plan_create_ex: unknown flags");
    LK_REQUIRE((flags & (LK_ALS_PLAN_REFERENCE_ORDER | LK_ALS_PLAN_HYBRID_ORDER)) !=
                   (LK_ALS_PLAN_REFERENCE_ORDER | LK_ALS_PLAN_HYBRID_ORDER),
               "lk_als_plan_create_ex: reference order is either strict or hybrid");
    LK_REQUIRE(n_rows >= 0 && n_rows < (int64_t)INT32_MAX, "lk_als_plan_create: bad n_rows");
    int KP = lk_padded_dim(k);
    LK_REQUIRE(KP > 0, "lk_als_plan_create: unsupported embedding size k=%d (1..1024)", k);
    if (solver == LK_SOLVER_AUTO) solver = LK_SOLVER_CHOLESKY;
    LK_REQUIRE(solver == LK_SOLVER_CHOLESKY || solver == LK_SOLVER_CG,
               "lk_als_plan_create: unknown solver %d", solver);
    LK_REQUIRE(!(solver == LK_SOLVER_CG && (KP < 64 || KP > 256)),
               "lk_als_plan_create: the CG solver serves 32 < k <= 256 (got %d)", k);
    LK_REQUIRE(!((flags & LK_ALS_PLAN_REFERENCE_ORDER) && KP > 256),
               "lk_als_plan_create_ex: reference-order plans stop at k = 256 (got %d)", k);

    auto *p = new lk_als_plan();
    p->n_rows = n_rows;
    p->k = k;
    p->KP = KP;
    p->NT = KP / 16;
    p->solver = solver;
    p->is64 = indptr_is_64 ? 1 : 0;
    p->cg_max_iter = 0;
    (void)hipGetDevice(&p->device);
    if (flags & LK_ALS_PLAN_REFERENCE_ORDER) {
        if (solver != LK_SOLVER_CHOLESKY) {
            delete p;
            lk::set_error("lk_als_plan_create_ex: reference order belongs to the exact solver");
            return LK_E_INVALID;
        }
        p->ref_order = true;
        p->chunk = 256;
        p->long_row = 256;
    }
    if ((flags & LK_ALS_PLAN_HYBRID_ORDER) && solver == LK_SOLVER_CHOLESKY && KP <= 256) {
        p->hybrid = true;
        p->chunk = 256;
        const char *e = getenv("LK_ALS_REF_LEN");
        int rl = e ? atoi(e) : LK_ALS_LONG_ROW;
        if (rl < 256) rl = 256;
        if (rl > LK_ALS_LONG_ROW) rl = LK_ALS_LONG_ROW;
        p->long_row = rl;
    }
    const int64_t CHUNK = p->chunk, LONG_ROW = KP > 256 ? INT64_MAX : (int64_t)p->long_row;

    auto len = [&](int64_t r) -> int64_t {
        if (indptr_is_64) {
            const int64_t *ip = static_cast<const int64_t *>(h_indptr);
            return ip[r + 1] - ip[r];
        }
        const int32_t *ip = static_cast<const int32_t *>(h_indptr);
        return (int64_t)ip[r + 1] - ip[r];
    };
    auto start = [&](int64_t r) -> int64_t {
        return indptr_is_64 ? static_cast<const int64_t *>(h_indptr)[r]
                            : (int64_t) static_cast<const int32_t *>(h_indptr)[r];
    };

    std::vector<int32_t> order((size_t)n_rows);
    {
        int64_t longest = 0;
        bool sane = true;
        for (int64_t r = 0; r < n_rows; ++r) {
            const int64_t n = len(r);
            if (n < 0) sane = false;
            if (n > longest) longest = n;
        }
        if (sane && longest <= 4 * n_rows + 65536) {
            std::vector<int64_t> at((size_t)longest + 2, 0);
            for (int64_t r = 0; r < n_rows; ++r) ++at[(size_t)len(r)];
            int64_t run = 0;
            for (int64_t n = longest; n >= 0; --n) {
                const int64_t c = at[(size_t)n];
                at[(size_t)n] = run;
                run += c;
            }
            for (int64_t r = 0; r < n_rows; ++r) order[(size_t)(at[(size_t)len(r)]++)] = (int32_t)r;
        } else {
            for (int64_t r = 0; r < n_rows; ++r) order[(size_t)r] = (int32_t)r;
            std::stable_sort(order.begin(), order.end(),
                             [&](int32_t x, int32_t y) { return len(x) > len(y); });
        }
    }

    auto first_at_most = [&](int64_t n, int64_t lo, int64_t hi) -> int64_t {
        return std::partition_point(order.begin() + lo, order.begin() + hi,
                                    [&](int32_t r) { return len(r) > n; }) -
               order.begin();
    };
    p->t_short = first_at_most(16, 0, n_rows);
    const int64_t t_8 = first_at_most(8, p->t_short, n_rows);
    const int64_t t_4 = first_at_most(4, t_8, n_rows);
    const int64_t t_64 = first_at_most(64, 0, p->t_short);
    const int64_t t_32 = first_at_most(32, t_64, p->t_short);
    const int64_t t_128 = first_at_most(128, 0, t_64);
    const int64_t cg_len = 16384 / KP;
    const int64_t t_cg = first_at_most(cg_len, 0, n_rows);
    p->t_cg1 = first_at_most(cg_len / 4, t_cg, n_rows);

    p->t_wb4 = switch_on("LK_ALS_WB4") ? t_4 : n_rows;
    p->t_wb8 = switch_on("LK_ALS_WB8") ? t_8 : p->t_wb4;
    const char *e_k128 = getenv("LK_ALS_WB64_K128");
    const int k128 = e_k128 ? atoi(e_k128) : LK_ALS_WB64_K128_DEFAULT;
    const int64_t t_wb = (KP == 256 || k128 >= 64) ? t_64 : (k128 >= 32 ? t_32 : p->t_short);
    p->wb_rows = n_rows - t_wb;
    const bool wb64 = switch_on("LK_ALS_WB64");
    p->t_wb64 = wb64 ? t_wb : p->t_short;
    const bool wb128 = KP == 256 && wb64 && switch_on("LK_ALS_WB128") && t_128 < t_64;
    p->t_wb128 = wb128 ? t_128 : p->t_wb64;
    p->side_streams = switch_on("LK_ALS_SIDE_STREAM");
    p->chunk_dma = KP == 256 && switch_on("LK_BLK_CHUNK_DMA");

    std::vector<int32_t> row_slab((size_t)n_rows, -1);
    std::vector<int32_t> chunk_row, chunk_slab;
    std::vector<int64_t> chunk_beg;
    std::vector<int32_t> chunk_len;
    p->unit = p->chunk;
    if (p->hybrid && (KP == 64 || p->chunk_dma)) {
        const char *e = getenv("LK_ALS_REF_UNIT");
        int u = e ? atoi(e) : LK_ALS_CHUNK;
        if (!e && KP == 64) {
            const int cus = device_cu_count(p->device);
            if (cus <= 0) {
                delete p;
                lk::set_error("lk_als_plan_create: cannot read the device's compute-unit count");
                return LK_E_HIP;
            }
            const int64_t want = 2 * (int64_t)cus * lk::als_chol_chunk_wgs_per_cu() * 4;
            int64_t units_1024 = 0, units_512 = 0;
            for (int64_t r = 0; r < n_rows; ++r) {
                const int64_t n = len(r);
                if (n > LONG_ROW) {
                    units_1024 += (n + 1023) / 1024;
                    units_512 += (n + 511) / 512;
                }
            }
            u = units_1024 >= want ? 1024 : (units_512 >= want ? 512 : 256);
        }
        if (u < p->chunk) u = p->chunk;
        p->unit = u / p->chunk * p->chunk;
    }
    const int64_t UNIT = p->unit;
    {
        for (int64_t r = 0; r < n_rows; ++r) {
            int64_t n = len(r);
            if (n > LONG_ROW) {
                row_slab[(size_t)r] = (int32_t)p->n_slabs;
                for (int64_t o = 0; o < n; o += UNIT) {
                    chunk_row.push_back((int32_t)r);
                    chunk_beg.push_back(start(r) + o);
                    chunk_len.push_back((int32_t)std::min<int64_t>(UNIT, n - o));
                    chunk_slab.push_back((int32_t)(p->n_slabs + o / CHUNK));
                }
                p->n_slabs += (n + CHUNK - 1) / CHUNK;
                p->n_long++;
            }
        }
    }
    if (p->n_slabs >= (int64_t)INT32_MAX) {
        delete p;
        lk::set_error("lk_als_plan_create: too many slabs");
        return LK_E_INVALID;
    }
    p->n_chunks = (int64_t)chunk_row.size();
    const char *e_cg = getenv("LK_ALS_CG_HYBRID");
    const int cg_mode = (e_cg && e_cg[0] >= '0' && e_cg[0] <= '2') ? e_cg[0] - '0' : 2;
    p->cg_exact = cg_mode == 2 ? t_cg : (cg_mode == 1 ? p->n_long : 0);
    std::vector<int32_t> grp_head, grp_cnt;
    for (int64_t r = 0; r < n_rows; ++r) {
        if (row_slab[(size_t)r] < 0) continue;
        const int64_t ns = (len(r) + CHUNK - 1) / CHUNK;
        if (p->ref_order || p->hybrid) {
            grp_head.push_back(row_slab[(size_t)r]);
            grp_cnt.push_back((int32_t)ns);
            continue;
        }
        if (ns <= LK_ALS_SLAB_GROUP) continue;
        for (int64_t s0 = 0; s0 < ns; s0 += LK_ALS_SLAB_GROUP) {
            const int64_t c = std::min<int64_t>(LK_ALS_SLAB_GROUP, ns - s0);
            if (c >= 2) {
                grp_head.push_back((int32_t)(row_slab[(size_t)r] + s0));
                grp_cnt.push_back((int32_t)c);
            }
        }
    }
    p->n_groups = (int64_t)grp_head.size();

    {
        auto padded = [](size_t bytes) { return lk::align_up(std::max<size_t>(bytes, 8), 256); };
        const size_t b_order = padded(order.size() * 4), b_rslab = padded(row_slab.size() * 4),
                     b_crow = padded(chunk_row.size() * 4), b_cbeg = padded(chunk_beg.size() * 8),
                     b_cslab = padded(chunk_slab.size() * 4), b_ghead = padded(grp_head.size() * 4),
                     b_gcnt = padded(grp_cnt.size() * 4), b_clen = padded(chunk_len.size() * 4);
        const size_t total = b_order + b_rslab + b_crow + b_cbeg + b_cslab + b_ghead + b_gcnt + b_clen;
        std::vector<char> host(total, 0);
        size_t o = 0;
        auto put = [&](const void *src, size_t bytes, size_t slot) {
            if (bytes) memcpy(host.data() + o, src, bytes);
            const size_t at = o;
            o += slot;
            return at;
        };
        const size_t o_order = put(order.data(), order.size() * 4, b_order);
        const size_t o_rslab = put(row_slab.data(), row_slab.size() * 4, b_rslab);
        const size_t o_cbeg = put(chunk_beg.data(), chunk_beg.size() * 8, b_cbeg);
        const size_t o_crow = put(chunk_row.data(), chunk_row.size() * 4, b_crow);
        const size_t o_cslab = put(chunk_slab.data(), chunk_slab.size() * 4, b_cslab);
        const size_t o_ghead = put(grp_head.data(), grp_head.size() * 4, b_ghead);
        const size_t o_gcnt = put(grp_cnt.data(), grp_cnt.size() * 4, b_gcnt);
        const size_t o_clen = put(chunk_len.data(), chunk_len.size() * 4, b_clen);
        hipError_t e = hipSuccess;
        p->d_pack = pack_pool_take(total, &p->pack_cap);
        if (!p->d_pack) {
            p->pack_cap = total;
            e = hipMalloc(reinterpret_cast<void **>(&p->d_pack), total);
        }
        if (e == hipSuccess) e = hipMemcpy(p->d_pack, host.data(), total, hipMemcpyHostToDevice);
        if (e != hipSuccess) {
            lk::set_error("lk_als_plan_create: %s", hipGetErrorString(e));
            lk_als_plan_destroy(p);
            return LK_E_HIP;
        }
        p->d_order = reinterpret_cast<int32_t *>(p->d_pack + o_order);
        p->d_row_slab = reinterpret_cast<int32_t *>(p->d_pack + o_rslab);
        p->d_chunk_beg = reinterpret_cast<int64_t *>(p->d_pack + o_cbeg);
        p->d_chunk_row = reinterpret_cast<int32_t *>(p->d_pack + o_crow);
        p->d_chunk_slab = reinterpret_cast<int32_t *>(p->d_pack + o_cslab);
        p->d_grp_head = reinterpret_cast<int32_t *>(p->d_pack + o_ghead);
        p->d_grp_cnt = reinterpret_cast<int32_t *>(p->d_pack + o_gcnt);
        p->d_chunk_len = reinterpret_cast<int32_t *>(p->d_pack + o_clen);
    }

    size_t off = 0;
    p->off_status = off;
    off += 256;
    p->off_otor = off;
    off += lk::align_up((size_t)KP * KP * sizeof(float), 256);
    p->off_delta = off;
    off += lk::align_up((size_t)std::max<int64_t>(n_rows, 1) * sizeof(float), 256);
    p->off_partial = off;
    off += lk::align_up((size_t)LK_DELTA_BLOCKS * sizeof(float), 256);
    p->off_slabs = off;
    if (KP > 256) {
        off += lk::align_up(lk::als_big_scratch_bytes(KP, n_rows), 256);
    } else {
        size_t slab_f = KP > 64 ? lk::als_blk_slab_floats(p->NT) : lk::als_chol_slab_floats(p->NT);
        off += lk::align_up((size_t)std::max<int64_t>(p->n_slabs, 1) * slab_f * sizeof(float),
                            256);
    }
    if (p->hybrid) {
        p->off_yref = off;
        off += lk::align_up((size_t)std::max<int64_t>(p->n_long, 1) * KP * sizeof(float), 256);
    }
    if (KP > 64 && KP <= 256) {
        p->off_ginv = off;
        off += lk::align_up((size_t)KP * KP * sizeof(float), 256);
        p->off_invws = off;
        off += lk::align_up(lk::spd_inverse_workspace_bytes(KP), 256);
    }
    p->ws_bytes = off;
    *out = p;
    return LK_OK;
}

extern "C" int lk_als_plan_enable_timing(lk_als_plan *p, int enable)
{
    LK_REQUIRE(p != nullptr, "lk_als_plan_enable_timing: null plan");
    if (enable && !p->ev[0][0]) {
        for (int i = 0; i < lk_als_plan::TIMING_RING; ++i)
            for (int j = 0; j < 3; ++j) LK_HIP_CHECK(hipEventCreate(&p->ev[i][j]));
    }
    p->timing = enable != 0;
    p->timing_n = 0;
    return LK_OK;
}

extern "C" int lk_als_plan_get_timing(lk_als_plan *p, double *ms_chunk, double *ms_solve,
                                      int32_t *n_launches)
{
    LK_REQUIRE(p && ms_chunk && ms_solve && n_launches, "lk_als_plan_get_timing: null pointer");
    *ms_chunk = 0.0;
    *ms_solve = 0.0;
    *n_launches = p->timing_n;
    for (int i = 0; i < p->timing_n; ++i) {
        float a = 0.f, b = 0.f;
        LK_HIP_CHECK(hipEventSynchronize(p->ev[i][2]));
        LK_HIP_CHECK(hipEventElapsedTime(&a, p->ev[i][0], p->ev[i][1]));
        LK_HIP_CHECK(hipEventElapsedTime(&b, p->ev[i][1], p->ev[i][2]));
        *ms_chunk += a;
        *ms_solve += b;
    }
    p->timing_n = 0;
    return LK_OK;
}

extern "C" void lk_als_plan_destroy(lk_als_plan *p)
{
    if (!p) return;
    int caller = -1;
    const bool swap = p->device >= 0 && hipGetDevice(&caller) == hipSuccess &&
                      caller != p->device && hipSetDevice(p->device) == hipSuccess;
    if (p->ev[0][0])
        for (int i = 0; i < lk_als_plan::TIMING_RING; ++i)
            for (int j = 0; j < 3; ++j) (void)hipEventDestroy(p->ev[i][j]);
    if (p->side) {
        (void)hipStreamSynchronize(p->side);
        lk::side_stream_release(p->side);
        (void)hipEventDestroy(p->ev_fork);
        (void)hipEventDestroy(p->ev_join);
    }
    if (p->side_rhs) {
        (void)hipStreamSynchronize(p->side_rhs);
        lk::side_stream_release(p->side_rhs);
        (void)hipEventDestroy(p->ev_fork_rhs);
        (void)hipEventDestroy(p->ev_join_rhs);
        (void)hipEventDestroy(p->ev_mid_rhs);
        (void)hipEventDestroy(p->ev_tail_rhs);
    }
    if (p->d_pack) {
        (void)hipDeviceSynchronize();
        if (!pack_pool_give(p->d_pack, p->pack_cap)) (void)hipFree(p->d_pack);
    }
    if (swap) (void)hipSetDevice(caller);
    delete p;
}

extern "C" size_t lk_als_plan_workspace_bytes(const lk_als_plan *p) { return p ? p->ws_bytes : 0; }
extern "C" int32_t lk_als_plan_solver(const lk_als_plan *p) { return p ? p->solver : -1; }

extern "C" int lk_als_plan_set_ctl(lk_als_plan *p, lk_task_ctl *ctl)
{
    LK_REQUIRE(p != nullptr, "lk_als_plan_set_ctl: null plan");
    p->ctl = ctl;
    return LK_OK;
}

extern "C" int64_t lk_als_plan_short_rows(const lk_als_plan *p)
{
    return p ? p->n_rows - p->t_short : 0;
}

extern "C" int64_t lk_als_plan_long_rows(const lk_als_plan *p) { return p ? p->n_long : 0; }
extern "C" int64_t lk_als_plan_units(const lk_als_plan *p) { return p ? p->n_chunks : 0; }
extern "C" int32_t lk_als_plan_unit(const lk_als_plan *p) { return p ? p->unit : 0; }

extern "C" const float *lk_als_plan_yref(const lk_als_plan *p, const void *d_ws)
{
    if (!p || !d_ws || !p->hybrid) return nullptr;
    return reinterpret_cast<const float *>(static_cast<const char *>(d_ws) + p->off_yref);
}

extern "C" int64_t lk_als_plan_woodbury_rows(const lk_als_plan *p) { return p ? p->wb_rows : 0; }

extern "C" int lk_als_plan_set_z(lk_als_plan *p, const float *d_z)
{
    LK_REQUIRE(p != nullptr, "lk_als_plan_set_z: null plan");
    p->d_z = d_z;
    return LK_OK;
}

extern "C" int lk_als_plan_set_z_shared(lk_als_plan *p, const float *d_z, const void *d_flag)
{
    LK_REQUIRE(p != nullptr, "lk_als_plan_set_z_shared: null plan");
    LK_REQUIRE((d_z == nullptr) == (d_flag == nullptr),
               "lk_als_plan_set_z_shared: Z and its flag word go together");
    LK_REQUIRE(d_z == nullptr || (p->KP > 64 && p->KP <= 256),
               "lk_als_plan_set_z_shared: the Woodbury kernels serve padded k = 128 / 256 only");
    p->d_z = d_z;
    p->d_zflag_src = static_cast<const int *>(d_flag);
    if (d_z) p->d_zbuf = nullptr;
    return LK_OK;
}

extern "C" int lk_als_plan_set_z_leader(lk_als_plan *p, int on)
{
    LK_REQUIRE(p != nullptr, "lk_als_plan_set_z_leader: null plan");
    p->z_for_others = on != 0;
    return LK_OK;
}

extern "C" const void *lk_als_plan_z_flag(const lk_als_plan *p, const void *d_ws)
{
    if (!p || !d_ws) return nullptr;
    return static_cast<const char *>(d_ws) + p->off_status + sizeof(int);
}

extern "C" int lk_als_plan_set_z_workspace(lk_als_plan *p, float *d_zbuf)
{
    LK_REQUIRE(p != nullptr, "lk_als_plan_set_z_workspace: null plan");
    LK_REQUIRE(d_zbuf == nullptr || (p->KP > 64 && p->KP <= 256),
               "lk_als_plan_set_z_workspace: the Woodbury kernels serve padded k = 128 / 256 only");
    p->d_zbuf = d_zbuf;
    if (d_zbuf) {
        p->d_z = nullptr;
        p->d_zflag_src = nullptr;
    }
    return LK_OK;
}

extern "C" int lk_als_plan_set_cg(lk_als_plan *p, float tol, int32_t max_iter)
{
    LK_REQUIRE(p != nullptr, "lk_als_plan_set_cg: null plan");
    LK_REQUIRE(tol > 0.f, "lk_als_plan_set_cg: tol must be positive");
    p->cg_tol = tol;
    p->cg_max_iter = max_iter;
    return LK_OK;
}

extern "C" int lk_als_plan_set_rhs_workspace(lk_als_plan *p, float *d_y)
{
    LK_REQUIRE(p != nullptr, "lk_als_plan_set_rhs_workspace: null plan");
    LK_REQUIRE(d_y == nullptr || p->solver == LK_SOLVER_CHOLESKY,
               "lk_als_plan_set_rhs_workspace: the reference-order right-hand side belongs to the "
               "exact solver (the CG option has no reference to reproduce)");
    p->d_yref = d_y;
    return LK_OK;
}

extern "C" int lk_als_implicit_half_epoch(const lk_als_plan *plan, const void *d_indptr,
                                          const int32_t *d_indices, const float *d_values,
                                          int64_t n_rows, int64_t n_cols, int32_t k,
                                          float *d_this, int32_t ld_this, const float *d_other,
                                          int32_t ld_other, const float *d_otor, int32_t ld_otor,
                                          void *d_ws, float *d_out_frob, void *stream)
{
    LK_REQUIRE(plan != nullptr, "lk_als_implicit_half_epoch: null plan");
    LK_REQUIRE(n_rows == plan->n_rows && k == plan->k,
               "lk_als_implicit_half_epoch: plan built for %lld rows, k=%d; got %lld rows, k=%d",
               (long long)plan->n_rows, plan->k, (long long)n_rows, k);
    LK_REQUIRE(ld_this == plan->KP && ld_other == plan->KP,
               "lk_als_implicit_half_epoch: factor leading dimensions (%d, %d) must equal "
               "lk_padded_dim(k)=%d",
               ld_this, ld_other, plan->KP);
    LK_REQUIRE(ld_otor >= k, "lk_als_implicit_half_epoch: ld_otor < k");
    LK_REQUIRE(d_indptr && d_this && d_otor && d_ws && d_out_frob,
               "lk_als_implicit_half_epoch: null pointer");
    LK_REQUIRE(n_cols >= 0 && (n_cols == 0 || d_other), "lk_als_implicit_half_epoch: null other");
    hipStream_t st = lk::as_stream(stream);
    char *ws = static_cast<char *>(d_ws);
    if (plan->solver == LK_SOLVER_CG)
        return lk::als_cg_half_epoch(plan, d_indptr, plan->is64, d_indices, d_values, n_rows, k,
                                     d_this, ld_this, d_other, ld_other, d_otor, ld_otor, ws,
                                     d_out_frob, st);
    if (plan->KP > 256)
        return lk::als_big_half_epoch(plan, d_indptr, plan->is64, d_indices, d_values, n_rows, k,
                                      d_this, d_other, d_otor, ld_otor, ws, d_out_frob, st, false,
                                      0.f);
    if (plan->KP > 64)
        return lk::als_blk_half_epoch(plan, d_indptr, plan->is64, d_indices, d_values, n_rows,
                                      n_cols, k, d_this, d_other, d_otor, ld_otor, ws, d_out_frob,
                                      st, false, 0.f);
    return lk::als_chol_half_epoch(plan, d_indptr, plan->is64, d_indices, d_values, n_rows, k,
                                   d_this, ld_this, d_other, ld_other, d_otor, ld_otor, ws,
                                   d_out_frob, st, false, 0.f);
}

extern "C" int lk_als_implicit_epoch(const lk_als_plan *user_plan, const lk_als_plan *item_plan,
                                     const void *d_u_indptr, const int32_t *d_u_indices,
                                     const float *d_u_values, const void *d_i_indptr,
                                     const int32_t *d_i_indices, const float *d_i_values,
                                     int32_t k, float *d_p, float *d_q, float *d_qtq,
                                     int32_t ld_qtq, float user_reg, float *d_ptp, int32_t ld_ptp,
                                     float item_reg, void *d_user_ws, void *d_item_ws,
                                     void *d_gram_ws, float *d_out_delta, void *stream)
{
    LK_REQUIRE(user_plan && item_plan, "lk_als_implicit_epoch: null plan");
    for (const lk_als_plan *p : {user_plan, item_plan})
        LK_REQUIRE(p->k == k && p->KP <= 64 && p->solver == LK_SOLVER_CHOLESKY && p->hybrid &&
                       !p->ctl && p->dense_limit < 0,
                   "lk_als_implicit_epoch serves hybrid-order plans of the exact solver at padded "
                   "k <= 64 without a task-control block (k=%d here); use the half-epoch calls",
                   k);
    LK_REQUIRE(user_plan != item_plan, "lk_als_implicit_epoch: one plan given twice");
    LK_REQUIRE(ld_qtq >= k && ld_ptp >= k, "lk_als_implicit_epoch: Gramian leading dimension < k");
    LK_REQUIRE(d_u_indptr && d_i_indptr && d_p && d_q && d_qtq && d_ptp && d_user_ws &&
                   d_item_ws && d_gram_ws && d_out_delta,
               "lk_als_implicit_epoch: null pointer");
    LK_REQUIRE(d_user_ws != d_item_ws && d_qtq != d_ptp,
               "lk_als_implicit_epoch: the two halves need buffers of their own");
    return lk::als_chol_epoch(user_plan, item_plan, d_u_indptr, d_u_indices, d_u_values,
                              d_i_indptr, d_i_indices, d_i_values, d_p, d_q, d_qtq, ld_qtq,
                              user_reg, d_ptp, ld_ptp, item_reg, static_cast<char *>(d_user_ws),
                              static_cast<char *>(d_item_ws), static_cast<float *>(d_gram_ws),
                              d_out_delta, lk::as_stream(stream));
}

extern "C" int lk_als_explicit_half_epoch(const lk_als_plan *plan, const void *d_indptr,
                                          const int32_t *d_indices, const float *d_values,
                                          int64_t n_rows, int64_t n_cols, int32_t k,
                                          float *d_this, int32_t ld_this, const float *d_other,
                                          int32_t ld_other, float reg, void *d_ws,
                                          float *d_out_frob, void *stream)
{
    LK_REQUIRE(plan != nullptr, "lk_als_explicit_half_epoch: null plan");
    LK_REQUIRE(n_rows == plan->n_rows && k == plan->k,
               "lk_als_explicit_half_epoch: plan built for %lld rows, k=%d; got %lld rows, k=%d",
               (long long)plan->n_rows, plan->k, (long long)n_rows, k);
    LK_REQUIRE(ld_this == plan->KP && ld_other == plan->KP,
               "lk_als_explicit_half_epoch: factor leading dimensions (%d, %d) must equal "
               "lk_padded_dim(k)=%d",
               ld_this, ld_other, plan->KP);
    LK_REQUIRE(d_indptr && d_this && d_ws && d_out_frob,
               "lk_als_explicit_half_epoch: null pointer");
    LK_REQUIRE(n_cols >= 0 && (n_cols == 0 || d_other), "lk_als_explicit_half_epoch: null other");
    LK_REQUIRE(plan->solver != LK_SOLVER_CG,
               "lk_als_explicit_half_epoch: only the exact (Cholesky) solver is built for the "
               "explicit model");
    hipStream_t st = lk::as_stream(stream);
    char *ws = static_cast<char *>(d_ws);
    if (plan->KP > 256)
        return lk::als_big_half_epoch(plan, d_indptr, plan->is64, d_indices, d_values, n_rows, k,
                                      d_this, d_other, nullptr, 0, ws, d_out_frob, st, true, reg);
    if (plan->KP > 64)
        return lk::als_blk_half_epoch(plan, d_indptr, plan->is64, d_indices, d_values, n_rows,
                                      n_cols, k, d_this, d_other, nullptr, 0, ws, d_out_frob, st,
                                      true, reg);
    return lk::als_chol_half_epoch(plan, d_indptr, plan->is64, d_indices, d_values, n_rows, k,
                                   d_this, ld_this, d_other, ld_other, nullptr, 0, ws, d_out_frob,
                                   st, true, reg);
}

extern "C" int lk_als_check_status(const lk_als_plan *plan, void *d_ws, void *stream)
{
    LK_REQUIRE(plan && d_ws, "lk_als_check_status: null pointer");
    int status[2] = {0, 0};
    LK_HIP_CHECK(hipMemcpyAsync(status, static_cast<char *>(d_ws) + plan->off_status,
                                sizeof(status), hipMemcpyDeviceToHost, lk::as_stream(stream)));
    LK_HIP_CHECK(hipStreamSynchronize(lk::as_stream(stream)));
    if (plan->ctl) {
        int rc = lk::ctl_finish(plan->ctl, lk::as_stream(stream));
        if (rc != LK_OK) return rc;
    }
    if (status[0] != 0) {
        lk::set_error("ALS solve error: normal matrix of row %d is not positive definite",
                      status[0] - 1);
        return LK_E_NOT_SPD;
    }
    return LK_OK;
}

namespace {
struct DevBuf {
    void *p = nullptr;
    ~DevBuf()
    {
        if (p) (void)hipFree(p);
    }
    int alloc(size_t bytes)
    {
        LK_HIP_CHECK(hipMalloc(&p, bytes ? bytes : 1));
        return LK_OK;
    }
};
}

extern "C" int lk_als_implicit_half_epoch_host_ctl(const void *h_indptr, int indptr_is_64,
                                                   const int32_t *h_indices,
                                                   const float *h_values, int64_t n_rows,
                                                   int64_t n_cols, int32_t k, float *h_this,
                                                   const float *h_other, const float *h_otor,
                                                   int32_t solver, float *h_out_frob,
                                                   lk_task_ctl *ctl)
{
    LK_REQUIRE(h_indptr && h_this && h_otor && h_out_frob, "half_epoch_host: null pointer");
    LK_REQUIRE(n_rows >= 0 && n_cols >= 0, "half_epoch_host: negative size");
    const int KP = lk_padded_dim(k);
    LK_REQUIRE(KP > 0, "half_epoch_host: unsupported k=%d", k);
    const int64_t nnz = indptr_is_64 ? static_cast<const int64_t *>(h_indptr)[n_rows]
                                     : static_cast<const int32_t *>(h_indptr)[n_rows];
    LK_REQUIRE(nnz >= 0 && (nnz == 0 || (h_indices && h_values && h_other)),
               "half_epoch_host: null pointer");
    lk_als_plan *plan = nullptr;
    int rc = lk_als_plan_create(&plan, h_indptr, indptr_is_64, n_rows, k, solver);
    if (rc != LK_OK) return rc;
    if (ctl && (rc = lk_als_plan_set_ctl(plan, ctl)) != LK_OK) {
        lk_als_plan_destroy(plan);
        return rc;
    }
    const size_t ipb = (size_t)(n_rows + 1) * (indptr_is_64 ? 8 : 4);
    DevBuf ip, idx, val, th, thp, ot, otp, oo, ws, fr, zb;
    auto fail = [&](int c) {
        lk_als_plan_destroy(plan);
        return c;
    };
    if ((rc = ip.alloc(ipb)) || (rc = idx.alloc((size_t)nnz * 4)) ||
        (rc = val.alloc((size_t)nnz * 4)) || (rc = th.alloc((size_t)n_rows * k * 4)) ||
        (rc = thp.alloc((size_t)n_rows * KP * 4)) || (rc = ot.alloc((size_t)n_cols * k * 4)) ||
        (rc = otp.alloc((size_t)n_cols * KP * 4)) || (rc = oo.alloc((size_t)k * k * 4)) ||
        (rc = ws.alloc(lk_als_plan_workspace_bytes(plan))) || (rc = fr.alloc(4)))
        return fail(rc);
    if (!ctl && KP > 64 && KP <= 256 && plan->solver == LK_SOLVER_CHOLESKY && n_cols > 0) {
        const char *e = getenv("LK_ALS_WB_MIN_ROWS");
        const int64_t wb_min = e ? atoll(e) : 4096;
        bool neg = false;
        for (int64_t i = 0; i < nnz && !neg; ++i) neg = h_values[i] < 0.f;
        if (wb_min > 0 && lk_als_plan_woodbury_rows(plan) >= wb_min && !neg) {
            if ((rc = zb.alloc((size_t)n_cols * KP * 4))) return fail(rc);
            if ((rc = lk_als_plan_set_z_workspace(plan, static_cast<float *>(zb.p)))) return fail(rc);
        }
    }
#define LK_H(expr)                                                              \
    do {                                                                        \
        hipError_t _e = (expr);                                                 \
        if (_e != hipSuccess) {                                                 \
            lk::set_error("%s failed: %s", #expr, hipGetErrorString(_e));       \
            return fail(LK_E_HIP);                                              \
        }                                                                       \
    } while (0)
    LK_H(hipMemcpy(ip.p, h_indptr, ipb, hipMemcpyHostToDevice));
    if (nnz > 0) {
        LK_H(hipMemcpy(idx.p, h_indices, (size_t)nnz * 4, hipMemcpyHostToDevice));
        LK_H(hipMemcpy(val.p, h_values, (size_t)nnz * 4, hipMemcpyHostToDevice));
    }
    if (n_rows > 0) LK_H(hipMemcpy(th.p, h_this, (size_t)n_rows * k * 4, hipMemcpyHostToDevice));
    if (n_cols > 0) LK_H(hipMemcpy(ot.p, h_other, (size_t)n_cols * k * 4, hipMemcpyHostToDevice));
    LK_H(hipMemcpy(oo.p, h_otor, (size_t)k * k * 4, hipMemcpyHostToDevice));
    if ((rc = lk_pad_rows((const float *)th.p, n_rows, k, k, (float *)thp.p, KP, nullptr)) ||
        (rc = lk_pad_rows((const float *)ot.p, n_cols, k, k, (float *)otp.p, KP, nullptr)))
        return fail(rc);
    rc = lk_als_implicit_half_epoch(plan, ip.p, (const int32_t *)idx.p, (const float *)val.p,
                                    n_rows, n_cols, k, (float *)thp.p, KP, (const float *)otp.p,
                                    KP, (const float *)oo.p, k, ws.p, (float *)fr.p, nullptr);
    if (rc != LK_OK) return fail(rc);
    const int rc_status = lk_als_check_status(plan, ws.p, nullptr);
    if (rc_status != LK_OK && rc_status != LK_E_CANCELLED) return fail(rc_status);
    if ((rc = lk_unpad_rows((const float *)thp.p, n_rows, k, KP, (float *)th.p, k, nullptr)))
        return fail(rc);
    LK_H(hipDeviceSynchronize());
    if (n_rows > 0) LK_H(hipMemcpy(h_this, th.p, (size_t)n_rows * k * 4, hipMemcpyDeviceToHost));
    LK_H(hipMemcpy(h_out_frob, fr.p, 4, hipMemcpyDeviceToHost));
#undef LK_H
    lk_als_plan_destroy(plan);
    return rc_status;
}

extern "C" int lk_als_implicit_half_epoch_host(const void *h_indptr, int indptr_is_64,
                                               const int32_t *h_indices, const float *h_values,
                                               int64_t n_rows, int64_t n_cols, int32_t k,
                                               float *h_this, const float *h_other,
                                               const float *h_otor, int32_t solver,
                                               float *h_out_frob)
{
    return lk_als_implicit_half_epoch_host_ctl(h_indptr, indptr_is_64, h_indices, h_values, n_rows,
                                               n_cols, k, h_this, h_other, h_otor, solver,
                                               h_out_frob, nullptr);
}
```

Before: 289.1 epochs/s.

## Use 32-bit SGPR-base DMA addressing, LDS-sourced y-chain, and reversed Cholesky L packing

Measured after the change: 303.4 epochs/s, median of 6. +4.9%, better.

```diff
diff --git a/lkpy_amd/csrc/als_cg.hip b/lkpy_amd/csrc/als_cg.hip
--- a/lkpy_amd/csrc/als_cg.hip
+++ b/lkpy_amd/csrc/als_cg.hip
@@ -462,9 +462,10 @@
         const int rc =
             p->KP > 64 ? als_blk_half_epoch(p, indptr, is64, indices, values, n_rows, 0, k, this_,
                                             other, otor, ld_otor, ws, out_frob, st, false, 0.f)
-                       : als_chol_half_epoch(p, indptr, is64, indices, values, n_rows, k, this_,
-                                             ld_this, other, ld_other, otor, ld_otor, ws, out_frob,
-                                             st, false, 0.f);
+                       : als_chol_half_epoch(p, indptr, is64, indices, values, n_rows,
+                                              -1, k, this_, ld_this, other,
+                                             ld_other, otor, ld_otor, ws, out_frob, st, false,
+                                             0.f);
         p->dense_limit = -1;
         if (rc != LK_OK) return rc;
         t_begin = t_exact;
diff --git a/lkpy_amd/csrc/als_chol.hip b/lkpy_amd/csrc/als_chol.hip
--- a/lkpy_amd/csrc/als_chol.hip
+++ b/lkpy_amd/csrc/als_chol.hip
@@ -213,22 +213,33 @@
     else wait_vm<0>();
 }
 
+template <bool WIDE>
 __device__ __forceinline__ void dma_issue(const unsigned ring_lds, const int slot_idx, const int g,
                                           const float *stage_slot,
                                           const float *__restrict__ other)
 {
     const int lane = lane_id();
     const unsigned col = __builtin_bit_cast(unsigned, stage_slot[g * 4]);
-    const uint64_t lane_base = (uint64_t)(uintptr_t)(other + (lane & 15) * 4);
-    const float *src = reinterpret_cast<const float *>(lane_base + (uint64_t)col * 256ull);
     const unsigned dst = ring_lds + slot_idx * 1024;
     unsigned keep;
-    asm volatile(
-        "s_mov_b32 %0, m0\n\ts_mov_b32 m0, %2\n\ts_nop 0\n\t"
-        "global_load_lds_dwordx4 %1, off\n\ts_mov_b32 m0, %0"
-        : "=&s"(keep)
-        : "v"(src), "s"(dst)
-        : "memory");
+    if constexpr (WIDE) {
+        const uint64_t lane_base = (uint64_t)(uintptr_t)(other + (lane & 15) * 4);
+        const float *src = reinterpret_cast<const float *>(lane_base + (uint64_t)col * 256ull);
+        asm volatile(
+            "s_mov_b32 %0, m0\n\ts_mov_b32 m0, %2\n\ts_nop 0\n\t"
+            "global_load_lds_dwordx4 %1, off\n\ts_mov_b32 m0, %0"
+            : "=&s"(keep)
+            : "v"(src), "s"(dst)
+            : "memory");
+    } else {
+        const unsigned off = col * 256u + (unsigned)(lane & 15) * 16u;
+        asm volatile(
+            "s_mov_b32 %0, m0\n\ts_mov_b32 m0, %2\n\ts_nop 0\n\t"
+            "global_load_lds_dwordx4 %1, %3\n\ts_mov_b32 m0, %0"
+            : "=&s"(keep)
+            : "v"(off), "s"(dst), "s"(other)
+            : "memory");
+    }
 }
 
 struct DmaOperand {
@@ -244,20 +255,45 @@
     return o;
 }
 
+template <bool MASKED>
+__device__ __forceinline__ void y_chain_lds(float &yc, const float *rows, const float *v1g,
+                                            const int g, const int nb)
+{
+    float q[4] = {rows[0], rows[64], rows[128], rows[192]};
+    const f32x4 v1 = *reinterpret_cast<const f32x4 *>(v1g);
+    if constexpr (MASKED) {
+#pragma unroll
+        for (int e = 0; e < 4; ++e) q[e] = (g * 4 + e) < nb ? q[e] : 0.f;
+    }
+    f32x2 lo = f32x2{q[0], q[1]} * f32x2{v1.x, v1.y};
+    f32x2 hi = f32x2{q[2], q[3]} * f32x2{v1.z, v1.w};
+    asm volatile("" : "+v"(lo), "+v"(hi));
+    yc = __fadd_rn(yc, lo.x);
+    yc = __fadd_rn(yc, lo.y);
+    yc = __fadd_rn(yc, hi.x);
+    yc = __fadd_rn(yc, hi.y);
+}
+
+struct DmaChain {
+    const float *rows = nullptr;
+    const float *v1 = nullptr;
+};
+
 template <bool MASKED, bool SEQY = false, bool WITH_Y = true>
 __device__ __forceinline__ void dma_apply(Gram<4> &G, const DmaOperand &o, const int g,
-                                          const int nb, const bool expl)
+                                          const int nb, const bool expl, const int slot_idx = 0,
+                                          const DmaChain ch = DmaChain{})
 {
     const int lane = lane_id();
     const bool live = !MASKED || (g * 4 + (lane >> 4)) < nb;
     const float v = o.v;
     const float va = expl ? 1.0f : v;
-    float q[4] = {o.q.x, o.q.y, o.q.z, o.q.w}, a[4];
-#pragma unroll
-    for (int t = 0; t < 4; ++t) {
-        q[t] = live ? q[t] : 0.f;
-        a[t] = q[t] * va;
-    }
+    float q[4] = {o.q.x, o.q.y, o.q.z, o.q.w};
+#pragma unroll
+    for (int t = 0; t < 4; ++t) q[t] = live ? q[t] : 0.f;
+    float a[4];
+#pragma unroll
+    for (int t = 0; t < 4; ++t) a[t] = q[t] * va;
 #pragma unroll
     for (int tj = 0; tj < 4; ++tj)
 #pragma unroll
@@ -265,10 +301,10 @@
             G.t[tidx(ti, tj)] = __builtin_amdgcn_mfma_f32_16x16x4f32(a[ti], q[tj],
                                                                      G.t[tidx(ti, tj)], 0, 0, 0);
     if constexpr (WITH_Y) {
-        const float v1 = expl ? v : v + 1.0f;
         if constexpr (SEQY) {
-            y_chain_step<4>(G.yc, q, v1);
+            y_chain_lds<MASKED>(G.yc, ch.rows + slot_idx * 256, ch.v1 + g * 4, g, nb);
         } else {
+            const float v1 = expl ? v : v + 1.0f;
 #pragma unroll
             for (int t = 0; t < 4; ++t) G.y[t] = fmaf(q[t], v1, G.y[t]);
         }
@@ -278,9 +314,10 @@
 template <bool MASKED, bool SEQY = false, bool WITH_Y = true>
 __device__ __forceinline__ void dma_consume(Gram<4> &G, const float *ring, const int slot_idx,
                                             const int g, const int nb, const float *stage_slot,
-                                            const bool expl)
-{
-    dma_apply<MASKED, SEQY, WITH_Y>(G, dma_fetch(ring, slot_idx, g, stage_slot), g, nb, expl);
+                                            const bool expl, const DmaChain ch = DmaChain{})
+{
+    dma_apply<MASKED, SEQY, WITH_Y>(G, dma_fetch(ring, slot_idx, g, stage_slot), g, nb, expl,
+                                    slot_idx, ch);
 }
 
 template <int NT>
@@ -290,12 +327,13 @@
 template <int NT, bool WITH_Y = true>
 __device__ __forceinline__ void gram_zero(Gram<NT> &G);
 
-template <bool SEQY = false, bool WITH_Y = true, int RING = DMA_RING>
+template <bool SEQY = false, bool WITH_Y = true, int RING = DMA_RING, bool WIDE = true>
 __device__ __forceinline__ void gram_accumulate_dma(Gram<4> &G, const int32_t *__restrict__ cols,
                                                     const float *__restrict__ vals, int64_t beg,
                                                     int64_t end, const float *__restrict__ other,
                                                     const bool expl, float *ring, float *stage,
-                                                    float *__restrict__ slab = nullptr)
+                                                    float *__restrict__ slab = nullptr,
+                                                    float *v1s = nullptr)
 {
     static_assert(RING == 8 || RING == 4, "DMA ring: 4 or 8 groups");
     const int lane = lane_id();
@@ -305,15 +343,20 @@
 
     float *wr_cur = stage + lane, *wr_nxt = stage + 128 + lane;
     const float *rd_cur = stage + (lane >> 4), *rd_nxt = stage + 128 + (lane >> 4);
+    DmaChain ch;
+    unsigned yb = 0;
+    if constexpr (SEQY && WITH_Y) ch.rows = ring + (lane & 15) * 4 + (lane >> 4);
     {
         const int64_t e = (beg + lane < end) ? beg + lane : last;
+        const float v = vals[e];
         wr_cur[0] = __builtin_bit_cast(float, cols[e]);
-        wr_cur[64] = vals[e];
+        wr_cur[64] = v;
+        if constexpr (SEQY && WITH_Y) v1s[lane] = expl ? v : v + 1.0f;
     }
     const int total = (int)((end - beg + 3) >> 2);
 #pragma unroll
     for (int g = 0; g < RING; ++g)
-        if (g < total) dma_issue(ring_lds, g, g, rd_cur, other);
+        if (g < total) dma_issue<WIDE>(ring_lds, g, g, rd_cur, other);
 
     int64_t base = beg;
     int g0 = 0;
@@ -327,6 +370,7 @@
         }
         wait_vm<RING - 1>();
         DmaOperand cur = dma_fetch(ring, 0, 0, rd_cur);
+        if constexpr (SEQY && WITH_Y) ch.v1 = v1s + yb;
 #pragma unroll
         for (int g = 0; g < 16; ++g) {
             DmaOperand nxt = cur;
@@ -334,15 +378,19 @@
                 wait_vm<RING - 2>();
                 nxt = dma_fetch(ring, (g + 1) % RING, g + 1, rd_cur);
             }
-            dma_apply<false, SEQY, WITH_Y>(G, cur, g, 64, expl);
+            dma_apply<false, SEQY, WITH_Y>(G, cur, g, 64, expl, g % RING, ch);
             if (g == 16 - RING - 2) {
                 wr_nxt[0] = __builtin_bit_cast(float, nxt_col);
                 wr_nxt[64] = nxt_val;
+                if constexpr (SEQY && WITH_Y) {
+                    asm volatile("" : "+v"(nxt_val));
+                    v1s[(yb ^ 64) + lane] = expl ? nxt_val : nxt_val + 1.0f;
+                }
             }
             if (g < 16 - RING)
-                dma_issue(ring_lds, g % RING, g + RING, rd_cur, other);
+                dma_issue<WIDE>(ring_lds, g % RING, g + RING, rd_cur, other);
             else
-                dma_issue(ring_lds, g % RING, g + RING - 16, rd_nxt, other);
+                dma_issue<WIDE>(ring_lds, g % RING, g + RING - 16, rd_nxt, other);
             cur = nxt;
             __builtin_amdgcn_sched_barrier(0);
         }
@@ -357,6 +405,7 @@
         const float *tr = rd_cur;
         rd_cur = rd_nxt;
         rd_nxt = tr;
+        yb ^= 64;
     }
     for (; g0 < total; base += 64, g0 += 16) {
         const int nb = (int)((end - base < 64) ? end - base : 64);
@@ -368,23 +417,28 @@
             nxt_col = cols[e];
             nxt_val = vals[e];
         }
+        if constexpr (SEQY && WITH_Y) ch.v1 = v1s + yb;
 #pragma unroll
         for (int g = 0; g < 16; ++g) {
             const int gg = g0 + g;
             if (gg < total) {
                 const int later = total - 1 - gg;
                 wait_vm_upto(later < RING - 1 ? later : RING - 1);
-                dma_consume<true, SEQY, WITH_Y>(G, ring, g % RING, g, nb, rd_cur, expl);
+                dma_consume<true, SEQY, WITH_Y>(G, ring, g % RING, g, nb, rd_cur, expl, ch);
             }
             if (g == 16 - RING - 2 && more) {
                 wr_nxt[0] = __builtin_bit_cast(float, nxt_col);
                 wr_nxt[64] = nxt_val;
+                if constexpr (SEQY && WITH_Y) {
+                    asm volatile("" : "+v"(nxt_val));
+                    v1s[(yb ^ 64) + lane] = expl ? nxt_val : nxt_val + 1.0f;
+                }
             }
             if (gg + RING < total) {
                 if (g < 16 - RING)
-                    dma_issue(ring_lds, g % RING, g + RING, rd_cur, other);
+                    dma_issue<WIDE>(ring_lds, g % RING, g + RING, rd_cur, other);
                 else
-                    dma_issue(ring_lds, g % RING, g + RING - 16, rd_nxt, other);
+                    dma_issue<WIDE>(ring_lds, g % RING, g + RING - 16, rd_nxt, other);
             }
         }
         if (slab && ((g0 + 16) & 63) == 0 && g0 + 16 < total) {
@@ -398,10 +452,11 @@
         const float *tr = rd_cur;
         rd_cur = rd_nxt;
         rd_nxt = tr;
-    }
-}
-
-template <bool WITH_Y = true, int RING = DMA_RING>
+        yb ^= 64;
+    }
+}
+
+template <bool WITH_Y = true, int RING = DMA_RING, bool WIDE = true>
 __device__ __forceinline__ void gram_accumulate_dma_256(Gram<4> &G, const int32_t *__restrict__ cols,
                                                         const float *__restrict__ vals, int64_t beg,
                                                         const float *__restrict__ other,
@@ -416,7 +471,7 @@
     wr0[0] = __builtin_bit_cast(float, cols[beg + lane]);
     wr0[64] = vals[beg + lane];
 #pragma unroll
-    for (int g = 0; g < RING; ++g) dma_issue(ring_lds, g, g, rd0, other);
+    for (int g = 0; g < RING; ++g) dma_issue<WIDE>(ring_lds, g, g, rd0, other);
 #pragma unroll
     for (int b = 0; b < 4; ++b) {
         float *const wr_nxt = (b & 1) ? wr0 : wr1;
@@ -449,9 +504,9 @@
             }
             if (gg + RING < TOTAL) {
                 if (g < 16 - RING)
-                    dma_issue(ring_lds, g % RING, g + RING, rd_cur, other);
+                    dma_issue<WIDE>(ring_lds, g % RING, g + RING, rd_cur, other);
                 else
-                    dma_issue(ring_lds, g % RING, g + RING - 16, rd_nxt, other);
+                    dma_issue<WIDE>(ring_lds, g % RING, g + RING - 16, rd_nxt, other);
             }
             cur = nxt;
             __builtin_amdgcn_sched_barrier(0);
@@ -560,7 +615,7 @@
     return by_lds < 5 ? by_lds : 5;
 }
 
-template <int NT, bool EXPL, bool WITH_Y>
+template <int NT, bool EXPL, bool WITH_Y, bool WIDE>
 __device__ __forceinline__ void als_chunk_body(
     const int32_t *__restrict__ indices, const float *__restrict__ values,
     const int64_t *__restrict__ chunk_beg, const int32_t *__restrict__ chunk_len,
@@ -581,16 +636,16 @@
     if constexpr (DMA) {
         const int len = chunk_len[c];
         if (block_len == 256 && len > 256) {
-            gram_accumulate_dma<false, WITH_Y, CHUNK_RING>(
+            gram_accumulate_dma<false, WITH_Y, CHUNK_RING, WIDE>(
                 G, indices, values, beg, beg + len, other, EXPL,
                 stage_all[wave] + GRAM_STAGE_WORDS, stage_all[wave], slab);
             slab += (size_t)((len - 1) >> 8) * slab_floats<NT>();
         } else if (len == 256)
-            gram_accumulate_dma_256<WITH_Y, CHUNK_RING>(
+            gram_accumulate_dma_256<WITH_Y, CHUNK_RING, WIDE>(
                 G, indices, values, beg, other, EXPL, stage_all[wave] + GRAM_STAGE_WORDS,
                 stage_all[wave]);
         else
-            gram_accumulate_dma<false, WITH_Y, CHUNK_RING>(
+            gram_accumulate_dma<false, WITH_Y, CHUNK_RING, WIDE>(
                 G, indices, values, beg, beg + len, other, EXPL,
                 stage_all[wave] + GRAM_STAGE_WORDS, stage_all[wave]);
     } else
@@ -599,7 +654,7 @@
     slab_store<NT, WITH_Y>(G, slab);
 }
 
-template <int NT, bool EXPL, bool WITH_Y>
+template <int NT, bool EXPL, bool WITH_Y, bool WIDE = false>
 __global__ __launch_bounds__(256) void als_chunk_kernel(
     const int32_t *__restrict__ indices, const float *__restrict__ values,
     const int64_t *__restrict__ chunk_beg, const int32_t *__restrict__ chunk_len,
@@ -607,20 +662,29 @@
     const int32_t *__restrict__ chunk_slab, int block_len)
 {
     __shared__ __attribute__((aligned(16))) float lds_flat[4 * chunk_lds_floats<NT>()];
-    als_chunk_body<NT, EXPL, WITH_Y>(indices, values, chunk_beg, chunk_len, n_chunks, other, ld,
+    als_chunk_body<NT, EXPL, WITH_Y, WIDE>(indices, values, chunk_beg, chunk_len, n_chunks, other, ld,
                                      slabs, (int64_t)blockIdx.x, lds_flat, chunk_slab, block_len);
 }
 
 template <int KP>
 struct LPack {
     __host__ __device__ static constexpr int c0(int j) { return (j + 1) & ~3; }
-    __host__ __device__ static constexpr int off(int j)
+    __host__ __device__ static constexpr int before(int j)
     {
         const int m = j >> 2, r = j & 3;
         return 4 * KP * m - 8 * m * m + 4 * m + r * (KP - 4 * m);
     }
     static constexpr int SIZE = KP * KP / 2 + KP;
+    static constexpr int RINV = 0, SCR = KP, IMG = KP + 256;
+    __host__ __device__ static constexpr int off(int j)
+    {
+        return IMG + SIZE - before(j) - (KP - c0(j));
+    }
 };
+static_assert(LPack<64>::off(62) - LPack<64>::c0(62) >= LPack<64>::SCR &&
+                  LPack<64>::off(0) + 64 == LPack<64>::IMG + LPack<64>::SIZE &&
+                  LPack<64>::off(63) == LPack<64>::IMG,
+              "L image: the stores of all 64 lanes stay between the scratch and the image's end");
 
 template <int NT>
 __host__ __device__ constexpr int hybrid_lds_floats()
@@ -635,8 +699,8 @@
     constexpr int KP = NT * 16, J = 4 * M, TJ = M >> 2, MG = M & 3;
     using P = LPack<KP>;
     const int slot = lane >> 4;
-    float *rinvarr = lds + P::SIZE;
-    float *scr = rinvarr + KP;
+    float *rinvarr = lds + P::RINV;
+    float *scr = lds + P::SCR;
 
 #pragma unroll
     for (int t = TJ; t < NT; ++t)
@@ -656,9 +720,13 @@
         rinvarr[j] = rinv;
         const float lj = (lane > j) ? pr[s0] * rinv : 0.f;
         if (j + 1 < KP) {
-            const bool in = lane >= P::c0(j) && lane < KP;
-            float *dst = in ? &lds[P::off(j) + lane - P::c0(j)] : &scr[lane];
-            *dst = lj;
+            if constexpr (KP == 64) {
+                lds[P::off(j) - P::c0(j) + lane] = lj;
+            } else {
+                const bool in = lane >= P::c0(j) && lane < KP;
+                float *dst = in ? &lds[P::off(j) + lane - P::c0(j)] : &scr[lane];
+                *dst = lj;
+            }
         }
         const float zj = bcast(b, j) * rinv;
         b = fmaf(-lj, zj, b);
@@ -712,7 +780,7 @@
     asm volatile("" : "+v"(b));
     *tmid = __builtin_amdgcn_s_memtime();
 #endif
-    const float dinv = (lane < KP) ? lds[P::SIZE + lane] : 0.f;
+    const float dinv = (lane < KP) ? lds[P::RINV + lane] : 0.f;
     b *= dinv;
     const int my_c0 = (lane + 1) & ~3;
     const float *mycol = lds + P::off(lane) - my_c0;
@@ -733,7 +801,7 @@
     return minpiv;
 }
 
-template <int NT, bool IS64, bool EXPL, bool CTL, bool YREF = false, bool SEQY = false>
+template <int NT, bool IS64, bool EXPL, bool CTL, bool YREF, bool SEQY, bool WIDE>
 __device__ __forceinline__ void als_solve_body(
     const typename IndPtr<IS64>::type *__restrict__ indptr, const int32_t *__restrict__ indices,
     const float *__restrict__ values, const int32_t *__restrict__ order, int64_t n_rows,
@@ -796,9 +864,12 @@
         for (int s = 0; s < ns; s += step)
             slab_add<NT, !YREF>(G, slabs + (size_t)(first_slab + s) * slab_floats<NT>());
     } else {
-        if constexpr (NT == 4)
-            gram_accumulate_dma<SEQY && !YREF>(G, indices, values, beg, end, other, EXPL, lds,
-                                               lds + LPack<KP>::SIZE + KP);
+        if constexpr (NT == 4) {
+            static_assert(NT != 4 || DMA_RING * 256 + 128 <= LPack<KP>::SIZE + KP, "v + 1 staging");
+            gram_accumulate_dma<SEQY && !YREF, true, DMA_RING, WIDE>(
+                G, indices, values, beg, end, other, EXPL, lds, lds + LPack<KP>::SIZE + KP,
+                nullptr, lds + DMA_RING * 256);
+        }
         else
             gram_accumulate<NT, SEQY && !YREF>(G, indices, values, beg, end, other, ld_other,
                                                EXPL, lds);
@@ -866,7 +937,8 @@
 #endif
 }
 
-template <int NT, bool IS64, bool EXPL, bool CTL, bool YREF = false, bool SEQY = false>
+template <int NT, bool IS64, bool EXPL, bool CTL, bool YREF = false, bool SEQY = false,
+          bool WIDE = false>
 __global__ __launch_bounds__(256) __attribute__((amdgpu_waves_per_eu(4))) void als_solve_kernel(
     const typename IndPtr<IS64>::type *__restrict__ indptr, const int32_t *__restrict__ indices,
     const float *__restrict__ values, const int32_t *__restrict__ order, int64_t n_rows,
@@ -877,7 +949,7 @@
     int chunk_rt = 0)
 {
     __shared__ __attribute__((aligned(16))) float lds_flat[4 * hybrid_lds_floats<NT>()];
-    als_solve_body<NT, IS64, EXPL, CTL, YREF, SEQY>(indptr, indices, values, order, n_rows,
+    als_solve_body<NT, IS64, EXPL, CTL, YREF, SEQY, WIDE>(indptr, indices, values, order, n_rows,
                                                     row_slab, other, ld_other, this_, ld_this,
                                                     otor_p, slabs, row_delta, status, k, reg, ctl,
                                                     y_ref, chunk_rt, (int64_t)blockIdx.x, lds_flat);
@@ -1144,6 +1216,12 @@
     float *yref = nullptr;
     bool tm = false;
     bool forked = false;
+    int64_t n_cols = -1;
+
+    bool wide() const
+    {
+        return n_cols < 0 || (uint64_t)n_cols * (uint64_t)ld_other * sizeof(float) >= (1ull << 32);
+    }
 
     int *status() const { return reinterpret_cast<int *>(ws + p->off_status); }
     float *otor_p() const { return reinterpret_cast<float *>(ws + p->off_otor); }
@@ -1195,17 +1273,26 @@
         h.forked = h.sr != st;
     }
     const bool chunk_y = !(h.yref != nullptr && h.n_y >= p->n_long);
+    constexpr bool CAN_WIDE = NT == 4;
+    const bool wide = CAN_WIDE && h.wide();
     if (p->n_chunks > 0) {
 #define LK_CHUNK_LAUNCH(WITHY)                                                                  \
-    hipLaunchKernelGGL((als_chunk_kernel<NT, EXPL, WITHY>),                                    \
+    if (wide)                                                                                  \
+        LK_CHUNK_LAUNCH_W(WITHY, CAN_WIDE);                                                    \
+    else                                                                                       \
+        LK_CHUNK_LAUNCH_W(WITHY, false)
+#define LK_CHUNK_LAUNCH_W(WITHY, WIDEV)                                                         \
+    hipLaunchKernelGGL((als_chunk_kernel<NT, EXPL, WITHY, WIDEV>),                             \
                        dim3((unsigned)((p->n_chunks + 3) / 4)), dim3(256), 0, st, h.indices,   \
                        h.values, p->d_chunk_beg, p->d_chunk_len, p->n_chunks, h.other,         \
                        h.ld_other, slabs, p->d_chunk_slab, p->unit > p->chunk ? (int)p->chunk : 0)
-        if (chunk_y)
+        if (chunk_y) {
             LK_CHUNK_LAUNCH(true);
-        else
+        } else {
             LK_CHUNK_LAUNCH(false);
+        }
 #undef LK_CHUNK_LAUNCH
+#undef LK_CHUNK_LAUNCH_W
     }
     if (h.n_y > 0) {
         int rc = launch_rhs_reference(p, h.indptr, IS64 ? 1 : 0, h.indices, h.values, p->d_order,
@@ -1238,11 +1325,20 @@
     const int ref_chunk = (p->ref_order || p->hybrid) ? p->chunk : 0;
     const int64_t n_y = h.n_y, n_solve = h.n_solve;
     float *yref = h.yref;
+    constexpr bool CAN_WIDE = NT == 4;
+    const bool wide = CAN_WIDE && h.wide();
     if (otor_ready) LK_HIP_CHECK(hipStreamWaitEvent(st, otor_ready, 0));
 #define LK_SOLVE_LAUNCH(CTLV, YREFV, T0, NTASKS, YPTR, STREAM)                                \
     LK_SOLVE_LAUNCH_S(CTLV, YREFV, false, T0, NTASKS, YPTR, STREAM)
 #define LK_SOLVE_LAUNCH_S(CTLV, YREFV, SEQV, T0, NTASKS, YPTR, STREAM)                        \
-    hipLaunchKernelGGL((als_solve_kernel<NT, IS64, EXPL, CTLV, YREFV, SEQV>),                  \
+    do {                                                                                       \
+        if (wide)                                                                              \
+            LK_SOLVE_LAUNCH_W(CTLV, YREFV, SEQV, CAN_WIDE, T0, NTASKS, YPTR, STREAM);          \
+        else                                                                                   \
+            LK_SOLVE_LAUNCH_W(CTLV, YREFV, SEQV, false, T0, NTASKS, YPTR, STREAM);             \
+    } while (0)
+#define LK_SOLVE_LAUNCH_W(CTLV, YREFV, SEQV, WIDEV, T0, NTASKS, YPTR, STREAM)                 \
+    hipLaunchKernelGGL((als_solve_kernel<NT, IS64, EXPL, CTLV, YREFV, SEQV, WIDEV>),           \
                        dim3((unsigned)(((NTASKS) + 3) / 4)), dim3(256), 0, (STREAM), ip,       \
                        h.indices, h.values, p->d_order + (T0), (NTASKS), p->d_row_slab,        \
                        h.other, h.ld_other, h.this_, h.ld_this, h.otor_p(), h.slabs(),         \
@@ -1278,6 +1374,7 @@
     }
 #undef LK_SOLVE_LAUNCH
 #undef LK_SOLVE_LAUNCH_S
+#undef LK_SOLVE_LAUNCH_W
     if (h.tm) {
         LK_HIP_CHECK(hipEventRecord(p->ev[p->timing_n][2], st));
         p->timing_n++;
@@ -1325,11 +1422,12 @@
 size_t als_chol_slab_floats(int NT) { return (size_t)(als_tiles(NT) * 4 + NT) * 64; }
 
 int als_chol_half_epoch(const lk_als_plan *p, const void *indptr, int is64, const int32_t *indices,
-                        const float *values, int64_t n_rows, int k, float *this_, int ld_this,
-                        const float *other, int ld_other, const float *otor, int ld_otor, char *ws,
-                        float *out_frob, hipStream_t st, bool expl, float reg)
+                        const float *values, int64_t n_rows, int64_t n_cols, int k, float *this_,
+                        int ld_this, const float *other, int ld_other, const float *otor,
+                        int ld_otor, char *ws, float *out_frob, hipStream_t st, bool expl, float reg)
 {
     CholHalf h{p, indptr, is64 != 0, indices, values, n_rows, k, this_, ld_this, other, ld_other, ws, reg, st};
+    h.n_cols = n_cols;
     int rc = half_prep(h, expl, otor, ld_otor);
     if (rc == LK_OK) rc = half_front(h, expl);
     if (rc == LK_OK) rc = half_solve(h, expl, nullptr);
@@ -1346,6 +1444,8 @@
     const int k = pu->k, KP = pu->KP;
     CholHalf hu{pu, u_indptr, pu->is64 != 0, u_indices, u_values, pu->n_rows, k, P, KP, Q, KP, ws_u, 0.f, st};
     CholHalf hi{pi, i_indptr, pi->is64 != 0, i_indices, i_values, pi->n_rows, k, Q, KP, P, KP, ws_i, 0.f, st};
+    hu.n_cols = pi->n_rows;
+    hi.n_cols = pu->n_rows;
     int rc = half_prep(hu, false, qtq, ld_qtq);
     if (rc == LK_OK) rc = half_front(hu, false);
     if (rc == LK_OK) rc = half_solve(hu, false, nullptr);
diff --git a/lkpy_amd/csrc/als_plan.h b/lkpy_amd/csrc/als_plan.h
--- a/lkpy_amd/csrc/als_plan.h
+++ b/lkpy_amd/csrc/als_plan.h
@@ -77,9 +77,9 @@
 namespace lk {
 size_t als_chol_slab_floats(int NT);
 int als_chol_half_epoch(const lk_als_plan *p, const void *indptr, int is64, const int32_t *indices,
-                        const float *values, int64_t n_rows, int k, float *this_, int ld_this,
-                        const float *other, int ld_other, const float *otor, int ld_otor, char *ws,
-                        float *out_frob, hipStream_t st, bool expl, float reg);
+                        const float *values, int64_t n_rows, int64_t n_cols, int k, float *this_,
+                        int ld_this, const float *other, int ld_other, const float *otor,
+                        int ld_otor, char *ws, float *out_frob, hipStream_t st, bool expl, float reg);
 size_t als_blk_slab_floats(int NT);
 int als_blk_half_epoch(const lk_als_plan *p, const void *indptr, int is64, const int32_t *indices,
                        const float *values, int64_t n_rows, int64_t n_cols, int k, float *this_,
diff --git a/lkpy_amd/csrc/als_plan.hip b/lkpy_amd/csrc/als_plan.hip
--- a/lkpy_amd/csrc/als_plan.hip
+++ b/lkpy_amd/csrc/als_plan.hip
@@ -608,8 +608,8 @@
         return lk::als_blk_half_epoch(plan, d_indptr, plan->is64, d_indices, d_values, n_rows,
                                       n_cols, k, d_this, d_other, d_otor, ld_otor, ws, d_out_frob,
                                       st, false, 0.f);
-    return lk::als_chol_half_epoch(plan, d_indptr, plan->is64, d_indices, d_values, n_rows, k,
-                                   d_this, ld_this, d_other, ld_other, d_otor, ld_otor, ws,
+    return lk::als_chol_half_epoch(plan, d_indptr, plan->is64, d_indices, d_values, n_rows, n_cols,
+                                   k, d_this, ld_this, d_other, ld_other, d_otor, ld_otor, ws,
                                    d_out_frob, st, false, 0.f);
 }
 
@@ -673,9 +673,9 @@
         return lk::als_blk_half_epoch(plan, d_indptr, plan->is64, d_indices, d_values, n_rows,
                                       n_cols, k, d_this, d_other, nullptr, 0, ws, d_out_frob, st,
                                       true, reg);
-    return lk::als_chol_half_epoch(plan, d_indptr, plan->is64, d_indices, d_values, n_rows, k,
-                                   d_this, ld_this, d_other, ld_other, nullptr, 0, ws, d_out_frob,
-                                   st, true, reg);
+    return lk::als_chol_half_epoch(plan, d_indptr, plan->is64, d_indices, d_values, n_rows, n_cols,
+                                   k, d_this, ld_this, d_other, ld_other, nullptr, 0, ws,
+                                   d_out_frob, st, true, reg);
 }
 
 extern "C" int lk_als_check_status(const lk_als_plan *plan, void *d_ws, void *stream)
```
